# Yaling-Li/DMA-YOLO

Measured on AMD Instinct MI355X. Metric: train images/sec (fwd+loss+bwd+optimizer, train.py batch loop) @1536; detect p50 ms incl. NMS, higher is better.
Workload: dtype bf16; 1 GPU; yolov5l-ca-sppfcspc-bifpn-scconv.yaml train @1536 nc=10; model=yolov5l-ca-sppfcspc-bifpn-scconv.yaml, global_batch=32, img=1536, parallelism=dp1

## Files before the change

### dma-yolo_amd/csrc/bn.hip

```cpp
#include "launch.h"

namespace {

template <typename T>
__global__ void bn_stats_kernel(const T* __restrict__ z, long zps, long M, int C, int rows_per_block,
                                float* __restrict__ psum, float* __restrict__ psq) {
  const int c = blockIdx.y * 64 + (threadIdx.x & 63);
  const int ty = threadIdx.x >> 6;
  __shared__ float s1[4][64], s2[4][64];
  float a = 0.f, b = 0.f;
  if (c < C) {
    const long r0 = (long)blockIdx.x * rows_per_block;
    const long r1 = min(M, r0 + rows_per_block);
#pragma unroll 8
    for (long m = r0 + ty; m < r1; m += 4) {
      float v = to_f(z[m * zps + c]);
      a += v;
      b += v * v;
    }
  }
  s1[ty][threadIdx.x & 63] = a;
  s2[ty][threadIdx.x & 63] = b;
  __syncthreads();
  if (ty == 0 && c < C) {
    const int l = threadIdx.x;
    psum[(long)blockIdx.x * C + c] = s1[0][l] + s1[1][l] + s1[2][l] + s1[3][l];
    psq[(long)blockIdx.x * C + c] = s2[0][l] + s2[1][l] + s2[2][l] + s2[3][l];
  }
}

__global__ void bn_finalize_kernel(const float* __restrict__ psum, const float* __restrict__ psq, int P, int C,
                                   double count, const float* __restrict__ gamma, const float* __restrict__ beta,
                                   float* __restrict__ rmean, float* __restrict__ rvar, long long* nbt, float momentum,
                                   float eps, int update, float* __restrict__ mean, float* __restrict__ invstd,
                                   float* __restrict__ scale, float* __restrict__ shift) {
  const int c = blockIdx.x;
  __shared__ double sa[256], sb[256];
  double a = 0.0, b = 0.0;
#pragma unroll 8
  for (int p = threadIdx.x; p < P; p += blockDim.x) {
    a += (double)psum[(long)p * C + c];
    b += (double)psq[(long)p * C + c];
  }
  sa[threadIdx.x] = a;
  sb[threadIdx.x] = b;
  __syncthreads();
  for (int s = blockDim.x / 2; s > 0; s >>= 1) {
    if ((int)threadIdx.x < s) {
      sa[threadIdx.x] += sa[threadIdx.x + s];
      sb[threadIdx.x] += sb[threadIdx.x + s];
    }
    __syncthreads();
  }
  if (threadIdx.x == 0) {
    const double mu = sa[0] / count;
    double var = sb[0] / count - mu * mu;
    if (var < 0) var = 0;
    const float is = (float)(1.0 / sqrt(var + (double)eps));
    mean[c] = (float)mu;
    invstd[c] = is;
    const float g = gamma ? gamma[c] : 1.f, bb = beta ? beta[c] : 0.f;
    scale[c] = g * is;
    shift[c] = bb - (float)mu * g * is;
    if (update) {
      const double unb = count > 1 ? var * count / (count - 1) : var;
      rmean[c] = (1.f - momentum) * rmean[c] + momentum * (float)mu;
      rvar[c] = (1.f - momentum) * rvar[c] + momentum * (float)unb;
      if (c == 0 && nbt) *nbt += 1;
    }
  }
}

__global__ void bn_eval_coef_kernel(const float* gamma, const float* beta, const float* rmean, const float* rvar,
                                    float eps, int C, float* scale, float* shift) {
  const int c = blockIdx.x * blockDim.x + threadIdx.x;
  if (c >= C) return;
  const float is = 1.f / sqrtf(rvar[c] + eps);
  const float g = gamma ? gamma[c] : 1.f, b = beta ? beta[c] : 0.f;
  scale[c] = g * is;
  shift[c] = b - rmean[c] * g * is;
}

struct RowMap {
  int cv, rr, RB, CV;
  DEV RowMap(int C, int VW) {
    CV = C / VW;
    RB = 256 / CV;
    cv = threadIdx.x % CV;
    rr = threadIdx.x / CV;
  }
  DEV bool active() const { return rr < RB; }
};

template <typename T, int U = 1>
__global__ void __launch_bounds__(256) bn_act_fwd_vec(const T* __restrict__ z, long zps, const float* __restrict__ scale,
                                                      const float* __restrict__ shift, int act, const T* __restrict__ res,
                                                      long rps, T* __restrict__ y, long yps, long M, int C, int rev) {
  constexpr int VW = Traits<T>::VW;
  RowMap rm(C, VW);
  if (!rm.active()) return;
  const int c0 = rm.cv * VW;
  float sc[VW], sh[VW];
  ldf<VW>(scale + c0, sc);
  ldf<VW>(shift + c0, sh);
  const long S = (long)gridDim.x * rm.RB;
  for (long m = (long)blockIdx.x * rm.RB + rm.rr; m < M; m += S * U) {
    uint4 zv[U], rv[U];
#pragma unroll
    for (int u = 0; u < U; ++u) {
      const long mu = rev ? M - 1 - (m + u * S) : m + u * S;
      if (m + u * S < M) {
        zv[u] = *reinterpret_cast<const uint4*>(z + mu * zps + c0);
        if (res) rv[u] = *reinterpret_cast<const uint4*>(res + mu * rps + c0);
      }
    }
#pragma unroll
    for (int u = 0; u < U; ++u) {
      const long mu = rev ? M - 1 - (m + u * S) : m + u * S;
      if (m + u * S >= M) break;
      float f[VW];
      unpack<T>(zv[u], f);
#pragma unroll
      for (int j = 0; j < VW; ++j) f[j] = f[j] * sc[j] + sh[j];
      act_fwd_n<VW>(act, f);
      if (res) {
        float r[VW];
        unpack<T>(rv[u], r);
#pragma unroll
        for (int j = 0; j < VW; ++j) f[j] += r[j];
      }
      *reinterpret_cast<uint4*>(y + mu * yps + c0) = pack<T>(f);
    }
  }
}

__global__ void __launch_bounds__(256) bn_act_fwd_f8_kernel(const bf16* __restrict__ z, long zps,
                                                            const float* __restrict__ scale,
                                                            const float* __restrict__ shift, int act,
                                                            const bf16* __restrict__ res, long rps, bf16* __restrict__ y,
                                                            long yps, long M, int C, unsigned char* __restrict__ y8,
                                                            const float* __restrict__ pmax, int G,
                                                            float* __restrict__ nmax, float* __restrict__ used,
                                                            float headroom, float* __restrict__ nsat) {
  __shared__ float red[4], rsat[4];
  float a = 0.f;
  for (int i = threadIdx.x; i < G; i += 256) a = nanmax(a, pmax[i]);
#pragma unroll
  for (int o = 32; o > 0; o >>= 1) a = nanmax(a, __shfl_xor(a, o, 64));
  if ((threadIdx.x & 63) == 0) red[threadIdx.x >> 6] = a;
  __syncthreads();
  a = nanmax(nanmax(red[0], red[1]), nanmax(red[2], red[3]));
  __syncthreads();
  a *= headroom;
  if (blockIdx.x == 0 && threadIdx.x == 0) used[0] = a;
  const float inv = a > 0.f ? 448.f / a : 1.f, thr = a > 0.f ? a : 448.f;
  RowMap rm(C, 8);
  float mx = 0.f, sat = 0.f;
  if (rm.active()) {
    const int c0 = rm.cv * 8;
    float sc[8], sh[8];
    ldf<8>(scale + c0, sc);
    ldf<8>(shift + c0, sh);
    for (long m = (long)blockIdx.x * rm.RB + rm.rr; m < M; m += (long)gridDim.x * rm.RB) {
      float f[8];
      unpack<bf16>(*reinterpret_cast<const uint4*>(z + m * zps + c0), f);
#pragma unroll
      for (int j = 0; j < 8; ++j) f[j] = f[j] * sc[j] + sh[j];
      act_fwd_n<8>(act, f);
      if (res) {
        float r[8];
        unpack<bf16>(*reinterpret_cast<const uint4*>(res + m * rps + c0), r);
#pragma unroll
        for (int j = 0; j < 8; ++j) f[j] += r[j];
      }
      const uint4 v = pack<bf16>(f);
      *reinterpret_cast<uint4*>(y + m * yps + c0) = v;
      unpack<bf16>(v, f);
#pragma unroll
      for (int j = 0; j < 8; ++j) {
        mx = nanmax(mx, fabsf(f[j]));
        sat += fabsf(f[j]) > thr ? 1.f : 0.f;
      }
      uint2 o;
      o.x = pack4_e4m3(f[0] * inv, f[1] * inv, f[2] * inv, f[3] * inv);
      o.y = pack4_e4m3(f[4] * inv, f[5] * inv, f[6] * inv, f[7] * inv);
      *reinterpret_cast<uint2*>(y8 + m * C + c0) = o;
    }
  }
#pragma unroll
  for (int o = 32; o > 0; o >>= 1) mx = nanmax(mx, __shfl_xor(mx, o, 64));
#pragma unroll
  for (int o = 32; o > 0; o >>= 1) sat += __shfl_xor(sat, o, 64);
  if ((threadIdx.x & 63) == 0) {
    red[threadIdx.x >> 6] = mx;
    rsat[threadIdx.x >> 6] = sat;
  }
  __syncthreads();
  if (threadIdx.x == 0) {
    nmax[blockIdx.x] = nanmax(nanmax(red[0], red[1]), nanmax(red[2], red[3]));
    if (nsat) nsat[blockIdx.x] = (rsat[0] + rsat[1]) + (rsat[2] + rsat[3]);
  }
}

template <typename T>
__global__ void bn_act_fwd_scalar(const T* __restrict__ z, long zps, const float* __restrict__ scale,
                                  const float* __restrict__ shift, int act, const T* __restrict__ res, long rps,
                                  T* __restrict__ y, long yps, long M, int C) {
  const long total = M * C;
  for (long i = blockIdx.x * (long)blockDim.x + threadIdx.x; i < total; i += (long)gridDim.x * blockDim.x) {
    const long m = i / C;
    const int c = (int)(i % C);
    float v = act_fwd(act, to_f(z[m * zps + c]) * scale[c] + shift[c]);
    if (res) v += to_f(res[m * rps + c]);
    y[m * yps + c] = from_f<T>(v);
  }
}

template <typename T, bool STATS, int U = 1>
__global__ void __launch_bounds__(256) bn_bwd_reduce_vec(const T* __restrict__ z, long zps, const T* __restrict__ dy,
                                                         long dps, const float* __restrict__ scale,
                                                         const float* __restrict__ shift, const float* __restrict__ mean,
                                                         const float* __restrict__ invstd, int act, long M, int C,
                                                         float* __restrict__ pdb, float* __restrict__ pdg, int rev) {
  constexpr int VW = Traits<T>::VW;
  __shared__ float red[2][256 * VW];
  RowMap rm(C, VW);
  const int c0 = rm.cv * VW;
  float a[VW], b[VW];
#pragma unroll
  for (int j = 0; j < VW; ++j) { a[j] = 0.f; b[j] = 0.f; }
  if (rm.active()) {
    float sc[VW], sh[VW], mu[VW], is[VW];
    if (STATS) {
#pragma unroll
      for (int j = 0; j < VW; ++j) {
        sc[j] = 1.f;
        sh[j] = 0.f;
        mu[j] = 0.f;
        is[j] = 1.f;
      }
    } else {
      ldf<VW>(scale + c0, sc);
      ldf<VW>(shift + c0, sh);
      ldf<VW>(mean + c0, mu);
      ldf<VW>(invstd + c0, is);
    }
    const long S = (long)gridDim.x * rm.RB;
    for (long m = (long)blockIdx.x * rm.RB + rm.rr; m < M; m += S * U) {
      uint4 zv[U], gv[U];
#pragma unroll
      for (int u = 0; u < U; ++u) {
        const long mu = rev ? M - 1 - (m + u * S) : m + u * S;
        if (m + u * S < M) {
          zv[u] = *reinterpret_cast<const uint4*>(z + mu * zps + c0);
          if (!STATS) gv[u] = *reinterpret_cast<const uint4*>(dy + mu * dps + c0);
        }
      }
#pragma unroll
      for (int u = 0; u < U; ++u) {
        if (m + u * S >= M) break;
        float zf[VW], gf[VW];
        unpack<T>(zv[u], zf);
        if (!STATS) unpack<T>(gv[u], gf);
        if (STATS) {
#pragma unroll
          for (int j = 0; j < VW; ++j) {
            a[j] += zf[j];
            b[j] += zf[j] * zf[j];
          }
        } else {
          float ag[VW];
#pragma unroll
          for (int j = 0; j < VW; ++j) ag[j] = zf[j] * sc[j] + sh[j];
          act_grad_n<VW>(act, ag);
#pragma unroll
          for (int j = 0; j < VW; ++j) {
            const float du = gf[j] * ag[j];
            a[j] += du;
            b[j] += du * (zf[j] - mu[j]) * is[j];
          }
        }
      }
    }
  }
#pragma unroll
  for (int j = 0; j < VW; ++j) {
    red[0][threadIdx.x * VW + j] = a[j];
    red[1][threadIdx.x * VW + j] = b[j];
  }
  __syncthreads();
  for (int c = threadIdx.x; c < C; c += blockDim.x) {
    const int cv = c / VW, j = c % VW;
    float s1 = 0.f, s2 = 0.f;
    for (int r = 0; r < rm.RB; ++r) {
      const int t = r * rm.CV + cv;
      s1 += red[0][t * VW + j];
      s2 += red[1][t * VW + j];
    }
    pdb[(long)blockIdx.x * C + c] = s1;
    pdg[(long)blockIdx.x * C + c] = s2;
  }
}

template <typename T, int U = 1>
__global__ void __launch_bounds__(256) bn_bwd_apply_vec(const T* __restrict__ z, long zps, const T* __restrict__ dy,
                                                        long dps, const float* __restrict__ scale,
                                                        const float* __restrict__ shift, const float* __restrict__ mean,
                                                        const float* __restrict__ invstd, int act,
                                                        const float* __restrict__ ca, const float* __restrict__ cb,
                                                        const float* __restrict__ cc, T* __restrict__ dz, long dzps,
                                                        long M, int C, int rev) {
  constexpr int VW = Traits<T>::VW;
  RowMap rm(C, VW);
  if (!rm.active()) return;
  const int c0 = rm.cv * VW;
  float sc[VW], sh[VW], k1[VW], k0[VW], k2[VW], t0[VW], t1[VW];
  ldf<VW>(scale + c0, sc);
  ldf<VW>(shift + c0, sh);
  ldf<VW>(ca + c0, k1);
  ldf<VW>(cc + c0, k2);
  ldf<VW>(invstd + c0, t0);
  ldf<VW>(cb + c0, k0);
  ldf<VW>(mean + c0, t1);
#pragma unroll
  for (int j = 0; j < VW; ++j) {
    k2[j] = k2[j] * t0[j];
    k0[j] = k0[j] - k2[j] * t1[j];
  }
  const long S = (long)gridDim.x * rm.RB;
  for (long m = (long)blockIdx.x * rm.RB + rm.rr; m < M; m += S * U) {
    uint4 zv[U], gv[U];
#pragma unroll
    for (int u = 0; u < U; ++u) {
      const long mu = rev ? M - 1 - (m + u * S) : m + u * S;
      if (m + u * S < M) {
        zv[u] = *reinterpret_cast<const uint4*>(z + mu * zps + c0);
        gv[u] = *reinterpret_cast<const uint4*>(dy + mu * dps + c0);
      }
    }
#pragma unroll
    for (int u = 0; u < U; ++u) {
      const long mu = rev ? M - 1 - (m + u * S) : m + u * S;
      if (m + u * S >= M) break;
      float zf[VW], gf[VW], o[VW];
      unpack<T>(zv[u], zf);
      unpack<T>(gv[u], gf);
#pragma unroll
      for (int j = 0; j < VW; ++j) o[j] = zf[j] * sc[j] + sh[j];
      act_grad_n<VW>(act, o);
#pragma unroll
      for (int j = 0; j < VW; ++j) o[j] = k1[j] * (gf[j] * o[j]) + k0[j] + k2[j] * zf[j];
      *reinterpret_cast<uint4*>(dz + mu * dzps + c0) = pack<T>(o);
    }
  }
}

template <typename T>
__global__ void bn_bwd_apply_scalar(const T* __restrict__ z, long zps, const T* __restrict__ dy, long dps,
                                    const float* __restrict__ scale, const float* __restrict__ shift,
                                    const float* __restrict__ mean, const float* __restrict__ invstd, int act,
                                    const float* __restrict__ ca, const float* __restrict__ cb,
                                    const float* __restrict__ cc, T* __restrict__ dz, long dzps, long M, int C) {
  const long total = M * C;
  for (long i = blockIdx.x * (long)blockDim.x + threadIdx.x; i < total; i += (long)gridDim.x * blockDim.x) {
    const long m = i / C;
    const int c = (int)(i % C);
    const float zv = to_f(z[m * zps + c]);
    const float du = to_f(dy[m * dps + c]) * act_grad(act, zv * scale[c] + shift[c]);
    dz[m * dzps + c] = from_f<T>(ca[c] * du + cb[c] + cc[c] * (zv - mean[c]) * invstd[c]);
  }
}

template <typename T>
__global__ void bn_bwd_reduce_kernel(const T* __restrict__ z, long zps, const T* __restrict__ dy, long dps,
                                     const float* __restrict__ scale, const float* __restrict__ shift,
                                     const float* __restrict__ mean, const float* __restrict__ invstd, int act,
                                     long M, int C, int rows_per_block, float* __restrict__ pdb,
                                     float* __restrict__ pdg) {
  const int c = blockIdx.y * 64 + (threadIdx.x & 63);
  const int ty = threadIdx.x >> 6;
  __shared__ float s1[4][64], s2[4][64];
  float a = 0.f, b = 0.f;
  if (c < C) {
    const float sc = scale[c], sh = shift[c], mu = mean[c], is = invstd[c];
    const long r0 = (long)blockIdx.x * rows_per_block;
    const long r1 = min(M, r0 + rows_per_block);
    for (long m = r0 + ty; m < r1; m += 4) {
      const float zv = to_f(z[m * zps + c]);
      const float du = to_f(dy[m * dps + c]) * act_grad(act, zv * sc + sh);
      a += du;
      b += du * (zv - mu) * is;
    }
  }
  s1[ty][threadIdx.x & 63] = a;
  s2[ty][threadIdx.x & 63] = b;
  __syncthreads();
  if (ty == 0 && c < C) {
    const int l = threadIdx.x;
    pdb[(long)blockIdx.x * C + c] = s1[0][l] + s1[1][l] + s1[2][l] + s1[3][l];
    pdg[(long)blockIdx.x * C + c] = s2[0][l] + s2[1][l] + s2[2][l] + s2[3][l];
  }
}

__global__ void bn_bwd_finalize_kernel(const float* __restrict__ pdb, const float* __restrict__ pdg, int P, int C,
                                       double count, const float* __restrict__ gamma, const float* __restrict__ invstd,
                                       float* __restrict__ dgamma, float* __restrict__ dbeta, float* __restrict__ ca,
                                       float* __restrict__ cb, float* __restrict__ cc) {
  const int c = blockIdx.x;
  __shared__ double sa[256], sb[256];
  double a = 0.0, b = 0.0;
#pragma unroll 8
  for (int p = threadIdx.x; p < P; p += blockDim.x) {
    a += (double)pdb[(long)p * C + c];
    b += (double)pdg[(long)p * C + c];
  }
  sa[threadIdx.x] = a;
  sb[threadIdx.x] = b;
  __syncthreads();
  for (int s = blockDim.x / 2; s > 0; s >>= 1) {
    if ((int)threadIdx.x < s) {
      sa[threadIdx.x] += sa[threadIdx.x + s];
      sb[threadIdx.x] += sb[threadIdx.x + s];
    }
    __syncthreads();
  }
  if (threadIdx.x == 0) {
    const float db = (float)sa[0], dg = (float)sb[0];
    if (dbeta) dbeta[c] = db;
    if (dgamma) dgamma[c] = dg;
    const float g = gamma ? gamma[c] : 1.f;
    const float k = g * invstd[c];
    ca[c] = k;
    cb[c] = (float)(-(double)k * sa[0] / count);
    cc[c] = (float)(-(double)k * sb[0] / count);
  }
}

__global__ void colsum2_kernel(const float* __restrict__ a, const float* __restrict__ b, long P, int C, int rows_per,
                               float* __restrict__ oa, float* __restrict__ ob) {
  const int c = blockIdx.y * 64 + (threadIdx.x & 63);
  const int ty = threadIdx.x >> 6;
  __shared__ double s1[4][64], s2[4][64];
  double x = 0.0, y = 0.0;
  if (c < C) {
    const long r0 = (long)blockIdx.x * rows_per, r1 = min(P, r0 + rows_per);
#pragma unroll 8
    for (long r = r0 + ty; r < r1; r += 4) {
      x += a[r * C + c];
      y += b[r * C + c];
    }
  }
  s1[ty][threadIdx.x & 63] = x;
  s2[ty][threadIdx.x & 63] = y;
  __syncthreads();
  if (ty == 0 && c < C) {
    const int l = threadIdx.x;
    oa[(long)blockIdx.x * C + c] = (float)(s1[0][l] + s1[1][l] + s1[2][l] + s1[3][l]);
    ob[(long)blockIdx.x * C + c] = (float)(s2[0][l] + s2[1][l] + s2[2][l] + s2[3][l]);
  }
}

}

constexpr int kRevAct = 1, kRevReduce = 0, kRevApply = 1;

DMY_API int dmy_bn_partial_rows(long M) {
  long p = (M + 255) / 256;
  return (int)(p < 1024 ? (p < 1 ? 1 : p) : 1024);
}

DMY_API int dmy_bn_stats(int dtype, const void* z, long zps, long M, int C, float* psum, float* psq, void* stream) {
  return by_dtype(dtype, kInvalid, [&](auto tag) {
    using T = typename decltype(tag)::type;
    constexpr int VW = Traits<T>::VW;
    hipStream_t st = (hipStream_t)stream;
    if (vec_ok(VW, C, {zps}, {}, {z}) && C / VW <= 256) {
      bn_bwd_reduce_vec<T, true><<<row_grid(M, C, VW, kRedCap), 256, 0, st>>>(
          (const T*)z, zps, (const T*)z, zps, nullptr, nullptr, nullptr, nullptr, 0, M, C, psum, psq, 0);
    } else {
      const int P = dmy_bn_partial_rows(M);
      const int rpb = (int)((M + P - 1) / P);
      bn_stats_kernel<T><<<dim3(P, ceil_div(C, 64)), 256, 0, st>>>((const T*)z, zps, M, C, rpb, psum, psq);
    }
    return (int)hipGetLastError();
  });
}

DMY_API int dmy_bn_finalize(const float* psum, const float* psq, int P, int C, double count, const float* gamma,
                            const float* beta, float* rmean, float* rvar, long long* nbt, float momentum, float eps,
                            int update, float* mean, float* invstd, float* scale, float* shift, void* stream) {
  bn_finalize_kernel<<<C, 256, 0, (hipStream_t)stream>>>(psum, psq, P, C, count, gamma, beta, rmean, rvar, nbt,
                                                         momentum, eps, update, mean, invstd, scale, shift);
  return (int)hipGetLastError();
}

DMY_API int dmy_bn_eval_coef(const float* gamma, const float* beta, const float* rmean, const float* rvar, float eps,
                             int C, float* scale, float* shift, void* stream) {
  bn_eval_coef_kernel<<<ceil_div(C, 256), 256, 0, (hipStream_t)stream>>>(gamma, beta, rmean, rvar, eps, C, scale, shift);
  return (int)hipGetLastError();
}


DMY_API int dmy_bn_act_fwd(int dtype, const void* z, long zps, const float* scale, const float* shift, int act,
                           const void* res, long rps, void* y, long yps, long M, int C, void* stream) {
  return by_dtype(dtype, kInvalid, [&](auto tag) {
    using T = typename decltype(tag)::type;
    constexpr int VW = Traits<T>::VW;
    hipStream_t st = (hipStream_t)stream;
    if (vec_ok(VW, C, {zps, yps, res ? rps : 0}, {}, {z, y, res}) && C / VW <= 256)
      bn_act_fwd_vec<T><<<row_grid(M, C, VW, kEwCap), 256, 0, st>>>((const T*)z, zps, scale, shift, act, (const T*)res, rps,
                                                                    (T*)y, yps, M, C, kRevAct);
    else
      bn_act_fwd_scalar<T><<<grid_cap(ceil_div(M * C, 256), 8192), 256, 0, st>>>((const T*)z, zps, scale, shift, act,
                                                                                 (const T*)res, rps, (T*)y, yps, M, C);
    return (int)hipGetLastError();
  });
}

DMY_API int dmy_bn_act_f8_blocks(void) { return 1024; }

DMY_API int dmy_bn_act_fwd_f8(const void* z, long zps, const float* scale, const float* shift, int act, const void* res,
                              long rps, void* y, long yps, long M, int C, void* y8, const float* pmax, float* nmax,
                              float* used, float headroom, float* nsat, void* stream) {
  if (C / 8 > 256 || !vec_ok(8, C, {zps, yps, res ? rps : 0}, {}, {z, y, res}) || ((uintptr_t)y8 & 7) || !(headroom >= 1.f))
    return kInvalid;
  const int G = dmy_bn_act_f8_blocks();
  bn_act_fwd_f8_kernel<<<G, 256, 0, (hipStream_t)stream>>>((const bf16*)z, zps, scale, shift, act, (const bf16*)res, rps,
                                                          (bf16*)y, yps, M, C, (unsigned char*)y8, pmax, G, nmax, used,
                                                          headroom, nsat);
  return (int)hipGetLastError();
}

DMY_API int dmy_bn_reduce_rows(int dtype, const void* z, long zps, const void* dy, long dps, long M, int C) {
  const int VW = vec_width(dtype);
  if (vec_ok(VW, C, {zps, dy ? dps : 0}, {}, {z, dy}) && C / VW <= 256) return row_grid(M, C, VW, kRedCap);
  return dmy_bn_partial_rows(M);
}

DMY_API int dmy_bn_bwd_reduce(int dtype, const void* z, long zps, const void* dy, long dps, const float* scale,
                              const float* shift, const float* mean, const float* invstd, int act, long M, int C,
                              float* pdb, float* pdg, void* stream) {
  return by_dtype(dtype, kInvalid, [&](auto tag) {
    using T = typename decltype(tag)::type;
    constexpr int VW = Traits<T>::VW;
    hipStream_t st = (hipStream_t)stream;
    if (vec_ok(VW, C, {zps, dps}, {}, {z, dy}) && C / VW <= 256) {
      bn_bwd_reduce_vec<T, false><<<row_grid(M, C, VW, kRedCap), 256, 0, st>>>(
          (const T*)z, zps, (const T*)dy, dps, scale, shift, mean, invstd, act, M, C, pdb, pdg, kRevReduce);
    } else {
      const int P = dmy_bn_partial_rows(M);
      const int rpb = (int)((M + P - 1) / P);
      bn_bwd_reduce_kernel<T><<<dim3(P, ceil_div(C, 64)), 256, 0, st>>>((const T*)z, zps, (const T*)dy, dps, scale, shift,
                                                                        mean, invstd, act, M, C, rpb, pdb, pdg);
    }
    return (int)hipGetLastError();
  });
}

DMY_API int dmy_colsum2_rows(long P) { return (int)(P < 256 ? P : 256); }

DMY_API int dmy_colsum2(const float* a, const float* b, long P, int C, float* oa, float* ob, void* stream) {
  const int S = dmy_colsum2_rows(P);
  const int rows = (int)((P + S - 1) / S);
  dim3 grid(S, ceil_div(C, 64));
  colsum2_kernel<<<grid, 256, 0, (hipStream_t)stream>>>(a, b, P, C, rows, oa, ob);
  return (int)hipGetLastError();
}

DMY_API int dmy_bn_bwd_finalize(const float* pdb, const float* pdg, int P, int C, double count, const float* gamma,
                                const float* invstd, float* dgamma, float* dbeta, float* ca, float* cb, float* cc,
                                void* stream) {
  bn_bwd_finalize_kernel<<<C, 256, 0, (hipStream_t)stream>>>(pdb, pdg, P, C, count, gamma, invstd, dgamma, dbeta, ca,
                                                             cb, cc);
  return (int)hipGetLastError();
}

DMY_API int dmy_bn_bwd_apply(int dtype, const void* z, long zps, const void* dy, long dps, const float* scale,
                             const float* shift, const float* mean, const float* invstd, int act, const float* ca,
                             const float* cb, const float* cc, void* dz, long dzps, long M, int C, void* stream) {
  return by_dtype(dtype, kInvalid, [&](auto tag) {
    using T = typename decltype(tag)::type;
    constexpr int VW = Traits<T>::VW;
    hipStream_t st = (hipStream_t)stream;
    if (vec_ok(VW, C, {zps, dps, dzps}, {}, {z, dy, dz}) && C / VW <= 256)
      bn_bwd_apply_vec<T><<<row_grid(M, C, VW, kEwCap), 256, 0, st>>>((const T*)z, zps, (const T*)dy, dps, scale, shift, mean,
                                                                      invstd, act, ca, cb, cc, (T*)dz, dzps, M, C, kRevApply);
    else
      bn_bwd_apply_scalar<T><<<grid_cap(ceil_div(M * C, 256), 8192), 256, 0, st>>>(
          (const T*)z, zps, (const T*)dy, dps, scale, shift, mean, invstd, act, ca, cb, cc, (T*)dz, dzps, M, C);
    return (int)hipGetLastError();
  });
}

__global__ void reduce_rows_kernel(const float* __restrict__ part, int P, int C, float* __restrict__ out, int acc) {
  const int c = blockIdx.x;
  __shared__ double s[256];
  double a = 0.0;
#pragma unroll 8
  for (int p = threadIdx.x; p < P; p += blockDim.x) a += (double)part[(long)p * C + c];
  s[threadIdx.x] = a;
  __syncthreads();
  for (int k = blockDim.x / 2; k > 0; k >>= 1) {
    if ((int)threadIdx.x < k) s[threadIdx.x] += s[threadIdx.x + k];
    __syncthreads();
  }
  if (threadIdx.x == 0) out[c] = (acc ? out[c] : 0.f) + (float)s[0];
}

DMY_API int dmy_reduce_rows(const float* part, int P, int C, float* out, int accumulate, void* stream) {
  reduce_rows_kernel<<<C, 256, 0, (hipStream_t)stream>>>(part, P, C, out, accumulate);
  return (int)hipGetLastError();
}

namespace {
DEV void pix_hwb(long m, int W, int H, bool small, int& w, int& h, int& b) {
  if (small) {
    const unsigned u = (unsigned)m, q = u / (unsigned)W;
    w = (int)(u - q * (unsigned)W);
    b = (int)(q / (unsigned)H);
    h = (int)(q - (unsigned)b * (unsigned)H);
  } else {
    w = (int)(m % W);
    h = (int)((m / W) % H);
    b = (int)(m / ((long)W * H));
  }
}

DEV int nearest_src_bn(int d, int in, int out) {
  if (out == in) return d;
  if (out == 2 * in) return d >> 1;
  const float scale = (float)in / (float)out;
  const int s = (int)floorf(__fmul_rn((float)d, scale));
  return s < in - 1 ? s : in - 1;
}

__global__ void __launch_bounds__(256) scgate_bn_fwd_kernel(const bf16* __restrict__ x, long xps,
                                                            const bf16* __restrict__ z, const float* __restrict__ scale,
                                                            const float* __restrict__ shift, const bf16* __restrict__ g,
                                                            bf16* __restrict__ out, int N, int H, int W, int C, int GH,
                                                            int GW) {
  constexpr int VW = 8;
  RowMap rm(C, VW);
  if (!rm.active()) return;
  const int c0 = rm.cv * VW;
  float sc[VW], sh[VW];
  ldf<VW>(scale + c0, sc);
  ldf<VW>(shift + c0, sh);
  const long M = (long)N * H * W, S = (long)gridDim.x * rm.RB;
  const bool small = M < (1L << 31);
  for (long m = (long)blockIdx.x * rm.RB + rm.rr; m < M; m += S) {
    int w, h, b;
    pix_hwb(m, W, H, small, w, h, b);
    const long gp = ((long)b * GH + nearest_src_bn(h, GH, H)) * GW + nearest_src_bn(w, GW, W);
    const uint4 xv = *reinterpret_cast<const uint4*>(x + m * xps + c0);
    const uint4 zv = *reinterpret_cast<const uint4*>(z + m * C + c0);
    const uint4 gv = *reinterpret_cast<const uint4*>(g + gp * C + c0);
    float xf[VW], zf[VW], gf[VW], o[VW];
    unpack<bf16>(xv, xf);
    unpack<bf16>(zv, zf);
    unpack<bf16>(gv, gf);
#pragma unroll
    for (int j = 0; j < VW; ++j) {
      const float u = to_f(from_f<bf16>(zf[j] * sc[j] + sh[j]));
      const float sg = sigmoidf_(to_f(from_f<bf16>(xf[j] + gf[j])));
      o[j] = u * to_f(from_f<bf16>(sg));
    }
    *reinterpret_cast<uint4*>(out + m * C + c0) = pack<bf16>(o);
  }
}

__global__ void __launch_bounds__(256) scgate_bn_bwd_kernel(
    const bf16* __restrict__ x, long xps, const bf16* __restrict__ z, const float* __restrict__ scale,
    const float* __restrict__ shift, const float* __restrict__ mean, const float* __restrict__ invstd,
    const bf16* __restrict__ g, const bf16* __restrict__ dout, bf16* __restrict__ du3, bf16* __restrict__ dpre, int N,
    int H, int W, int C, int GH, int GW, float* __restrict__ pdb, float* __restrict__ pdg) {
  constexpr int VW = 8;
  __shared__ float red[2][256 * VW];
  RowMap rm(C, VW);
  const int c0 = rm.cv * VW;
  float a[VW], bsum[VW];
#pragma unroll
  for (int j = 0; j < VW; ++j) a[j] = bsum[j] = 0.f;
  if (rm.active()) {
    float sc[VW], sh[VW], mu[VW], is[VW];
    ldf<VW>(scale + c0, sc);
    ldf<VW>(shift + c0, sh);
    ldf<VW>(mean + c0, mu);
    ldf<VW>(invstd + c0, is);
    const long M = (long)N * H * W, S = (long)gridDim.x * rm.RB;
    const bool small = M < (1L << 31);
    for (long m = (long)blockIdx.x * rm.RB + rm.rr; m < M; m += S) {
      int w, h, b;
      pix_hwb(m, W, H, small, w, h, b);
      const long gp = ((long)b * GH + nearest_src_bn(h, GH, H)) * GW + nearest_src_bn(w, GW, W);
      const uint4 xv = *reinterpret_cast<const uint4*>(x + m * xps + c0);
      const uint4 zv = *reinterpret_cast<const uint4*>(z + m * C + c0);
      const uint4 gv = *reinterpret_cast<const uint4*>(g + gp * C + c0);
      const uint4 dv = *reinterpret_cast<const uint4*>(dout + m * C + c0);
      float xf[VW], zf[VW], gf[VW], df[VW], du[VW], dp[VW];
      unpack<bf16>(xv, xf);
      unpack<bf16>(zv, zf);
      unpack<bf16>(gv, gf);
      unpack<bf16>(dv, df);
#pragma unroll
      for (int j = 0; j < VW; ++j) {
        const float u = to_f(from_f<bf16>(zf[j] * sc[j] + sh[j]));
        const float sg = sigmoidf_(to_f(from_f<bf16>(xf[j] + gf[j])));
        dp[j] = df[j] * u * sg * (1.f - sg);
        du[j] = df[j] * sg;
      }
      const uint4 duv = pack<bf16>(du);
      *reinterpret_cast<uint4*>(du3 + m * C + c0) = duv;
      *reinterpret_cast<uint4*>(dpre + m * C + c0) = pack<bf16>(dp);
      float dr[VW];
      unpack<bf16>(duv, dr);
#pragma unroll
      for (int j = 0; j < VW; ++j) {
        a[j] += dr[j];
        bsum[j] += dr[j] * (zf[j] - mu[j]) * is[j];
      }
    }
  }
#pragma unroll
  for (int j = 0; j < VW; ++j) {
    red[0][threadIdx.x * VW + j] = a[j];
// ... 44 lines not shown
```

### dma-yolo_amd/csrc/bwd1x1.hip

```cpp
#include "launch.h"

namespace {
namespace b1 {

constexpr unsigned kOob = 0xFFFFFFF0u;

DEV __amdgpu_buffer_rsrc_t rsrc(const void* base, unsigned bytes) {
  return __builtin_amdgcn_make_buffer_rsrc(const_cast<void*>(base), 0, (int)bytes, 0x00020000);
}
DEV uint4 bload(__amdgpu_buffer_rsrc_t r, unsigned off) {
  const auto v = __builtin_amdgcn_raw_buffer_load_b128(r, off, 0, 0);
  return *reinterpret_cast<const uint4*>(&v);
}

template <int ROW> DEV int ksw(int k, int row) {
  constexpr int RB = ROW * 2;
  const int c = row >> 3, w = row & 7;
  int key;
  if constexpr (RB >= 256) key = 2 * ((k & 3) | (((k >> 3) & 1) << 2));
  else key = 2 * (((k >> 1) & 1) | (((k >> 3) & 1) << 1));
  return k * ROW + (((c ^ key) & (ROW / 8 - 1)) << 3) + w;
}
template <int K> DEV int wsw(int r, int ch) {
  if constexpr (K * 2 >= 256) return (ch ^ (r & 15)) & (K / 8 - 1);
  else return (ch ^ ((r >> 1) & 7)) & (K / 8 - 1);
}
template <int ROW> DEV bf16x8 frag_t(const bf16* base, int r0, int k0, int lane) {
  typedef short s4 __attribute__((ext_vector_type(4)));
  const int g = lane >> 4, il = lane & 15, q = il >> 2, p = il & 3;
  const bf16* a0 = base + ksw<ROW>(k0 + 8 * g + q, r0 + 4 * p);
  const bf16* a1 = base + ksw<ROW>(k0 + 8 * g + 4 + q, r0 + 4 * p);
  const s4 lo = __builtin_amdgcn_ds_read_tr16_b64_v4i16((__attribute__((address_space(3))) s4*)(a0));
  const s4 hi = __builtin_amdgcn_ds_read_tr16_b64_v4i16((__attribute__((address_space(3))) s4*)(a1));
  bf16x8 r;
  r[0] = lo[0]; r[1] = lo[1]; r[2] = lo[2]; r[3] = lo[3];
  r[4] = hi[0]; r[5] = hi[1]; r[6] = hi[2]; r[7] = hi[3];
  return r;
}
DEV unsigned pk2(float a, float b) {
  const bf16 x = __float2bfloat16(a), y = __float2bfloat16(b);
  return (unsigned)*reinterpret_cast<const unsigned short*>(&x) |
         ((unsigned)*reinterpret_cast<const unsigned short*>(&y) << 16);
}

template <int K, int CB, int TP, int PX>
struct Shape {
  static constexpr int NT = 256, KCH = K / 8, CCH = CB / 8;
  static constexpr int NDZ = TP * KCH / NT, NX = TP * CCH / NT;
  static constexpr int RDZ = NT / KCH, RXS = NT / CCH;
  static constexpr int KW = K / 2, CW = CB / 2, MI = KW / 16, NJ = CW / 16;
  static constexpr int PGN = TP / (16 * PX), U = PGN * (CB / 64), UPW = (U + 3) / 4;
  static constexpr int LDS = (CB * K + TP * K + TP * CB) * 2;
  static_assert(K % 64 == 0 && CB % 64 == 0 && NT % KCH == 0 && NT % CCH == 0, "channels");
  static_assert(NDZ >= 1 && NX >= 1 && TP % 32 == 0 && TP % (16 * PX) == 0 && U >= 1, "tile");
  static_assert(LDS <= 160 * 1024, "LDS");
};

template <int K, int CB, int TP, int PX>
__global__ void __launch_bounds__(256, 1) conv1x1_bwd_bn(
    const bf16* __restrict__ dy, long dps, const bf16* __restrict__ z, const bf16* __restrict__ x, long xps,
    const bf16* __restrict__ wt, const float* __restrict__ scale, const float* __restrict__ shift,
    const float* __restrict__ mean, const float* __restrict__ invstd, int act, const float* __restrict__ ca,
    const float* __restrict__ cb, const float* __restrict__ cc, bf16* __restrict__ dx, long bps, int accumulate,
    float* __restrict__ dw, float* __restrict__ dws, long M, int ntiles, int C, int nsplit, unsigned dyb, unsigned zb,
    unsigned xb) {
  using S = Shape<K, CB, TP, PX>;
  extern __shared__ __attribute__((aligned(16))) char b1_smem[];
  bf16* ws = reinterpret_cast<bf16*>(b1_smem);
  bf16* dzs = ws + CB * K;
  bf16* xs = dzs + TP * K;
  const int tid = threadIdx.x, lane = tid & 63, wid = tid >> 6, g = lane >> 4, il = lane & 15;
  const int slot = blockIdx.x >> 3, cs = slot % nsplit;
  const int grp = (blockIdx.x & 7) + 8 * (slot / nsplit), ngrp = gridDim.x / nsplit;
  const int cbase = cs * CB;
  x += cbase;
  dx += cbase;
  dw += cbase;

  for (int e = tid; e < CB * S::KCH; e += S::NT) {
    const int r = e / S::KCH, ch = e % S::KCH;
    *reinterpret_cast<uint4*>(ws + r * K + (wsw<K>(r, ch) << 3)) =
        *reinterpret_cast<const uint4*>(wt + (long)(cbase + r) * K + ch * 8);
  }

  const int kc8 = (tid % S::KCH) * 8, xc8 = (tid % S::CCH) * 8;
  float sc[8], sh[8], k1[8], k0[8], k2[8];
  {
    float t0[8], t1[8];
    ldf<8>(scale + kc8, sc);
    ldf<8>(shift + kc8, sh);
    ldf<8>(ca + kc8, k1);
    ldf<8>(cc + kc8, k2);
    ldf<8>(invstd + kc8, t0);
    ldf<8>(cb + kc8, k0);
    ldf<8>(mean + kc8, t1);
#pragma unroll
    for (int j = 0; j < 8; ++j) {
      k2[j] = k2[j] * t0[j];
      k0[j] = k0[j] - k2[j] * t1[j];
    }
  }

  const __amdgpu_buffer_rsrc_t rdy = rsrc(dy, dyb), rz = rsrc(z, zb), rx = rsrc(x, xb - 2u * cbase);
  uint4 pg[S::NDZ], pz[S::NDZ], pxv[S::NX];
  auto issue = [&](int t) {
    const long m0 = (long)t * TP;
#pragma unroll
    for (int j = 0; j < S::NDZ; ++j) {
      const long m = m0 + tid / S::KCH + j * S::RDZ;
      const bool ok = m < M;
      pg[j] = bload(rdy, ok ? (unsigned)((m * dps + kc8) * 2) : kOob);
      pz[j] = bload(rz, ok ? (unsigned)((m * K + kc8) * 2) : kOob);
    }
#pragma unroll
    for (int j = 0; j < S::NX; ++j) {
      const long m = m0 + tid / S::CCH + j * S::RXS;
      pxv[j] = bload(rx, m < M ? (unsigned)((m * xps + xc8) * 2) : kOob);
    }
  };

  f32x4 wacc[S::MI][S::NJ];
#pragma unroll
  for (int i = 0; i < S::MI; ++i)
#pragma unroll
    for (int j = 0; j < S::NJ; ++j) wacc[i][j] = f32x4{0.f, 0.f, 0.f, 0.f};
  const int wk = wid >> 1, wc = wid & 1;
  const int chq = (g & 1) * 16 + (g >> 1) * 8;

  int t = grp;
  if (t < ntiles) issue(t);
  __syncthreads();
  for (; t < ntiles; t += ngrp) {
    const long m0 = (long)t * TP;
#pragma unroll
    for (int j = 0; j < S::NDZ; ++j) {
      float zf[8], gf[8], o[8];
      unpack<bf16>(pz[j], zf);
      unpack<bf16>(pg[j], gf);
#pragma unroll
      for (int e = 0; e < 8; ++e) o[e] = zf[e] * sc[e] + sh[e];
      act_grad_n<8>(act, o);
#pragma unroll
      for (int e = 0; e < 8; ++e) o[e] = k1[e] * (gf[e] * o[e]) + k0[e] + k2[e] * zf[e];
      pg[j] = pack<bf16>(o);
    }
    __syncthreads();
#pragma unroll
    for (int j = 0; j < S::NDZ; ++j)
      *reinterpret_cast<uint4*>(dzs + ksw<K>(tid / S::KCH + j * S::RDZ, kc8)) = pg[j];
#pragma unroll
    for (int j = 0; j < S::NX; ++j)
      *reinterpret_cast<uint4*>(xs + ksw<CB>(tid / S::CCH + j * S::RXS, xc8)) = pxv[j];
    __syncthreads();

    uint4 old[S::UPW][PX][2];
    if (accumulate) {
#pragma unroll
      for (int s = 0; s < S::UPW; ++s) {
        const int u = wid + 4 * s, p0 = (u % S::PGN) * 16 * PX, c0 = (u / S::PGN) * 64;
        if (u >= S::U) break;
#pragma unroll
        for (int pt = 0; pt < PX; ++pt) {
          const long m = m0 + p0 + pt * 16 + il;
#pragma unroll
          for (int h = 0; h < 2; ++h)
            old[s][pt][h] = m < M ? *reinterpret_cast<const uint4*>(dx + m * bps + c0 + h * 32 + chq)
                                  : make_uint4(0, 0, 0, 0);
        }
      }
    }
    if (t + ngrp < ntiles) issue(t + ngrp);

#pragma unroll
    for (int s = 0; s < S::UPW; ++s) {
      const int u = wid + 4 * s, p0 = (u % S::PGN) * 16 * PX, c0 = (u / S::PGN) * 64;
      if (u >= S::U) break;
      f32x4 acc[4][PX];
#pragma unroll
      for (int ct = 0; ct < 4; ++ct)
#pragma unroll
        for (int pt = 0; pt < PX; ++pt) acc[ct][pt] = f32x4{0.f, 0.f, 0.f, 0.f};
#pragma unroll 2
      for (int kc = 0; kc < K / 32; ++kc) {
        bf16x8 b[PX];
#pragma unroll
        for (int pt = 0; pt < PX; ++pt)
          b[pt] = *reinterpret_cast<const bf16x8*>(dzs + ksw<K>(p0 + pt * 16 + il, kc * 32 + 8 * g));
#pragma unroll
        for (int ct = 0; ct < 4; ++ct) {
          const int r = c0 + ct * 16 + il;
          const bf16x8 a = *reinterpret_cast<const bf16x8*>(ws + r * K + (wsw<K>(r, kc * 4 + g) << 3));
#pragma unroll
          for (int pt = 0; pt < PX; ++pt)
            acc[ct][pt] = __builtin_amdgcn_mfma_f32_16x16x32_bf16(a, b[pt], acc[ct][pt], 0, 0, 0);
        }
      }
#pragma unroll
      for (int pt = 0; pt < PX; ++pt) {
        const long m = m0 + p0 + pt * 16 + il;
#pragma unroll
        for (int h = 0; h < 2; ++h) {
          const f32x4 &a = acc[2 * h][pt], &b = acc[2 * h + 1][pt];
          const auto s0 = __builtin_amdgcn_permlane16_swap(pk2(a[0], a[1]), pk2(b[0], b[1]), false, false);
          const auto s1 = __builtin_amdgcn_permlane16_swap(pk2(a[2], a[3]), pk2(b[2], b[3]), false, false);
          uint4 v;
          v.x = s0[0];
          v.y = s1[0];
          v.z = s0[1];
          v.w = s1[1];
          if (accumulate) {
            float f[8], o[8];
            unpack<bf16>(v, f);
            unpack<bf16>(old[s][pt][h], o);
#pragma unroll
            for (int j = 0; j < 8; ++j) f[j] += o[j];
            v = pack<bf16>(f);
          }
          if (m < M) *reinterpret_cast<uint4*>(dx + m * bps + c0 + h * 32 + chq) = v;
        }
      }
    }

#pragma unroll
    for (int ps = 0; ps < TP / 32; ++ps) {
      bf16x8 a[S::MI];
#pragma unroll
      for (int i = 0; i < S::MI; ++i) a[i] = frag_t<K>(dzs, wk * S::KW + i * 16, ps * 32, lane);
#pragma unroll
      for (int j = 0; j < S::NJ; ++j) {
        const bf16x8 b = frag_t<CB>(xs, wc * S::CW + j * 16, ps * 32, lane);
#pragma unroll
        for (int i = 0; i < S::MI; ++i)
          wacc[i][j] = __builtin_amdgcn_mfma_f32_16x16x32_bf16(a[i], b, wacc[i][j], 0, 0, 0);
      }
    }
  }
  float* part = dws != nullptr ? dws + (long)blockIdx.x * K * CB : nullptr;
#pragma unroll
  for (int i = 0; i < S::MI; ++i)
#pragma unroll
    for (int j = 0; j < S::NJ; ++j)
#pragma unroll
      for (int r = 0; r < 4; ++r) {
        const int kk = wk * S::KW + i * 16 + 4 * g + r, c = wc * S::CW + j * 16 + il;
        if (part != nullptr) part[kk * CB + c] = wacc[i][j][r];
        else atomicAdd(dw + (long)kk * C + c, wacc[i][j][r]);
      }
}

__global__ void __launch_bounds__(256) wgrad_slots_reduce(const float* __restrict__ dws, float* __restrict__ dw, int K,
                                                          int C, int CB, int nblocks, int nsplit) {
  const long e = (long)blockIdx.x * blockDim.x + threadIdx.x;
  if (e >= (long)K * C) return;
  const int k = (int)(e / C), c = (int)(e % C), cs = c / CB, cl = c % CB;
  float s = 0.f;
  for (int b = 0; b < nblocks; ++b)
    if (((b >> 3) % nsplit) == cs) s += dws[((long)b * K + k) * CB + cl];
  dw[e] += s;
}

int num_cus() {
  static int n = 0;
  if (n == 0) {
    int dev = 0;
    (void)hipGetDevice(&dev);
    if (hipDeviceGetAttribute(&n, hipDeviceAttributeMultiprocessorCount, dev) != hipSuccess || n <= 0) n = 256;
  }
  return n;
}

struct Plan {
  int cb, tp, px;
};
constexpr Plan plan(int K, int C) {
  return (K == 64 && C == 64) ? Plan{64, 128, 2} : (K == 128 && C == 64) ? Plan{64, 128, 2}
       : (K == 64 && C == 128) ? Plan{128, 64, 2} : (K == 128 && C == 128) ? Plan{128, 64, 2}
       : (K == 128 && C == 256) ? Plan{256, 64, 2} : (K == 128 && C == 512) ? Plan{256, 64, 2}
       : (K == 256 && C == 256) ? Plan{128, 32, 1} : (K == 256 && C == 128) ? Plan{128, 32, 1}
       : (K == 64 && C == 256) ? Plan{256, 64, 2} : Plan{0, 0, 0};
}

inline int grid_blocks(long M, int K, int C) {
  const Plan pl = plan(K, C);
  const int ns = C / pl.cb, ntiles = ceil_div(M, pl.tp);
  int ngrp = num_cus() / ns;
  if (ngrp > ntiles) ngrp = (ntiles + 7) / 8 * 8;
  return ngrp * ns;
}

template <int K, int C>
int launch(const bf16* dy, long dps, const bf16* z, const bf16* x, long xps, const bf16* wt, const float* scale,
           const float* shift, const float* mean, const float* invstd, int act, const float* ca, const float* cb,
           const float* cc, bf16* dx, long bps, int acc, float* dw, float* ws, long M, hipStream_t st) {
  constexpr Plan pl = plan(K, C);
  constexpr int CB = pl.cb, TP = pl.tp, PX = pl.px, NS = C / CB;
  using S = Shape<K, CB, TP, PX>;
  static bool raised = false;
  if (!raised) {
    (void)hipFuncSetAttribute((const void*)conv1x1_bwd_bn<K, CB, TP, PX>,
                              hipFuncAttributeMaxDynamicSharedMemorySize, S::LDS);
    raised = true;
  }
  const int nb = grid_blocks(M, K, C);
  conv1x1_bwd_bn<K, CB, TP, PX><<<nb, 256, S::LDS, st>>>(
      dy, dps, z, x, xps, wt, scale, shift, mean, invstd, act, ca, cb, cc, dx, bps, acc, dw, ws, M, ceil_div(M, TP), C,
      NS, (unsigned)(2.0 * (double)M * dps), (unsigned)(2.0 * (double)M * K), (unsigned)(2.0 * (double)M * xps));
  if (ws != nullptr)
    wgrad_slots_reduce<<<ceil_div((long)K * C, 256), 256, 0, st>>>(ws, dw, K, C, CB, nb, NS);
  return (int)hipGetLastError();
}
}
}

DMY_API int dmy_conv1x1_bwd_bn_ok(long M, int K, int C, long dps, long xps, long bps, const void* dy, const void* z,
                                  const void* x, const void* dx) {
  if (b1::plan(K, C).cb == 0 || M <= 0) return 0;
  if (!vec_ok(8, 0, {dps, xps, bps}, {}, {dy, z, x, dx}) || dps < K || xps < C || bps < C) return 0;
  const double lim = (double)b1::kOob - 64.0;
  if (2.0 * (double)M * dps >= lim || 2.0 * (double)M * K >= lim || 2.0 * (double)M * xps >= lim) return 0;
  return 1;
}

DMY_API long dmy_conv1x1_bwd_bn_ws_elems(long M, int K, int C) {
  if (b1::plan(K, C).cb == 0 || M <= 0) return 0;
  return (long)b1::grid_blocks(M, K, C) * K * b1::plan(K, C).cb;
}

DMY_API int dmy_conv1x1_bwd_bn(const void* dy, long dps, const void* z, const void* x, long xps, const void* wt,
                               const float* scale, const float* shift, const float* mean, const float* invstd, int act,
                               const float* ca, const float* cb, const float* cc, void* dx, long bps, int accumulate,
                               float* dw, float* ws, long ws_elems, long M, int K, int C, void* stream) {
  if (!dmy_conv1x1_bwd_bn_ok(M, K, C, dps, xps, bps, dy, z, x, dx)) return -1;
  if (ws != nullptr && ws_elems < dmy_conv1x1_bwd_bn_ws_elems(M, K, C)) return -1;
  hipStream_t st = (hipStream_t)stream;
#define B1_GO(K_, C_)                                                                                                 \
  if (K == K_ && C == C_)                                                                                            \
    return b1::launch<K_, C_>((const bf16*)dy, dps, (const bf16*)z, (const bf16*)x, xps, (const bf16*)wt, scale,     \
                              shift, mean, invstd, act, ca, cb, cc, (bf16*)dx, bps, accumulate, dw, ws, M, st);
  B1_GO(64, 64)
  B1_GO(128, 64)
  B1_GO(64, 128)
  B1_GO(128, 128)
  B1_GO(128, 256)
  B1_GO(128, 512)
  B1_GO(256, 128)
  B1_GO(256, 256)
  B1_GO(64, 256)
#undef B1_GO
  return -1;
}
```

### dma-yolo_amd/dmayolo/_lib.py

```python
import ctypes
import os

import torch

_HERE = os.path.dirname(os.path.abspath(__file__))
LIB_PATH = os.path.join(_HERE, 'libdmayolo_hip.so')
if os.environ.get('DMY_LIB_AB'):
    LIB_PATH = os.path.join(_HERE, os.path.basename(os.environ['DMY_LIB_AB']))

P, I, L, F, D = ctypes.c_void_p, ctypes.c_int, ctypes.c_long, ctypes.c_float, ctypes.c_double

SIGNATURES = {
    'dmy_conv_fwd_partial_rows': [L, I],
    'dmy_conv_fwd_bound_rows': [L, I],
    'dmy_conv_fwd_last_rows': [],
    'dmy_conv_fwd_bn_rows': [I, P, P, P, P, I, I, I, I, L, I, I, I, I, I, I, I, L],
    'dmy_conv_fwd': [I, P, P, P, P, P, P, I, I, I, I, L, I, I, I, I, I, I, I, L, P],
    'dmy_conv_dgrad': [I, P, P, P, I, I, I, I, I, L, I, I, I, I, I, I, I, L, P],
    'dmy_conv_fwd_act': [I, P, P, P, P, I, I, I, I, L, I, I, I, I, I, I, I, L, P, P, I, P, L, P],
    'dmy_conv_fwd_splitk_elems': [I, P, P, P, I, I, I, I, L, I, I, I, I, I, I, I, L],
    'dmy_conv_fwd_act_ws': [I, P, P, P, P, I, I, I, I, L, I, I, I, I, I, I, I, L, P, P, I, P, L, P, L, P],
    'dmy_conv_route': [I, I, P, P, P, I, I, I, I, L, I, I, I, I, I, I, I, L, I],
    'dmy_conv_wgrad': [I, P, P, P, I, I, I, I, L, I, I, I, I, I, I, I, L, P],
    'dmy_conv_wprep_multi': [I, P, I, P],
    'dmy_conv_wprep_s2d': [I, P, P, I, I, I, P],
    'dmy_conv_wgrad_s2d_to_oihw': [P, P, I, I, I, P],
    'dmy_image_s2d': [I, I, P, P, I, I, I, I, I, F, P],
    'dmy_conv_wgrad_ex': [I, P, P, P, I, I, I, I, L, I, I, I, I, I, I, I, L, I, P],
    'dmy_conv_wgrad_ws_elems': [I, P, P, I, I, I, I, L, I, I, I, I, I, I, I, L, I],
    'dmy_conv_wgrad_det': [I, P, P, P, I, I, I, I, L, I, I, I, I, I, I, I, L, I, P, L, P],
    'dmy_conv_wprep': [I, P, P, P, I, I, I, I, I, P],
    'dmy_dwconv_ok': [I, P, P, P, I, I, I, I, I, I, L, I, I, I, I, I, I, L],
    'dmy_dwconv_fwd_rows': [L, I],
    'dmy_dwconv_fwd': [I, P, P, P, P, P, P, I, I, I, I, L, I, I, I, I, I, I, L, P],
    'dmy_dwconv_fwd_act': [I, P, P, P, P, I, I, I, I, L, I, I, I, I, I, I, L, P, P, I, P, L, P],
    'dmy_dwconv_dgrad': [I, P, P, P, I, I, I, I, I, L, I, I, I, I, I, I, L, P],
    'dmy_dwconv_wgrad_rows': [L, I],
    'dmy_dwconv_wgrad': [I, P, P, P, I, I, I, I, L, I, I, I, I, I, I, L, P],
    'dmy_dwconv_wgrad_finalize': [P, I, I, I, I, P, I, P],
    'dmy_dwconv_wgrad_bias': [I, P, P, P, I, I, I, I, L, I, I, I, I, I, I, L, P],
    'dmy_dwconv_wgrad_bias_finalize': [P, I, I, I, I, P, I, P, I, P],
    'dmy_dwconv_fwd_actbn': [I, P, P, P, P, I, I, I, I, L, I, I, I, I, I, I, L, P, P, I, P, L, P],
    'dmy_actbn_stats': [I, P, L, I, L, I, P, P, P],
    'dmy_actbn_fwd': [I, P, L, I, P, P, P, L, P, L, L, I, P],
    'dmy_actbn_bwd_reduce': [I, P, L, P, L, P, P, I, L, I, P, P, P],
    'dmy_actbn_bwd_apply': [I, P, L, P, L, P, P, I, P, P, P, P, L, L, I, P, P],
    'dmy_adapt_gate_blocks': [I, L, I, I],
    'dmy_adapt_gate_fwd': [I, I, P, L, I, P, L, I, P, L, I, P, L, P, P, P, L, P, L, P],
    'dmy_adapt_gate_bwd': [I, I, P, L, P, L, I, P, L, I, P, L, I, P, P, L, P, P, L, P, L, P, L, I, P, L, P, P, L, P],
    'dmy_adapt_add_fwd': [I, I, P, L, P, L, P, L, P, F, P, L, L, I, P],
    'dmy_adapt_add_bwd': [I, I, P, L, P, L, P, L, P, L, P, F, P, L, P, L, P, L, I, P, L, I, P],
    'dmy_conv1x1_bwd_bn_ok': [L, I, I, L, L, L, P, P, P, P],
    'dmy_conv1x1_bwd_bn': [P, L, P, P, L, P, P, P, P, P, I, P, P, P, P, L, I, P, P, L, L, I, I, P],
    'dmy_conv1x1_bwd_bn_ws_elems': [L, I, I],
    'dmy_aug_desc_bytes': [],
    'dmy_augment_batch': [P, I, P, I, I, P],
    'dmy_mosaic_desc_bytes': [],
    'dmy_mosaic_compose': [P, I, I, P],
    'dmy_letterbox_desc_bytes': [],
    'dmy_letterbox_batch': [I, P, P, I, P, I, I, I, I, F, P],
    'dmy_scale_boxes': [P, P, P, P, P, P, I, I, P],
    'dmy_fp8_quant_ws_elems': [],
    'dmy_fp8_quant': [P, L, I, L, P, P, P],
    'dmy_conv_wprep_fp8': [P, P, P, I, I, I, I, P],
    'dmy_conv_fwd_fp8_partial_rows': [L, I],
    'dmy_conv_fwd_fp8': [P, P, P, P, P, P, P, P, I, I, I, I, I, I, I, I, I, I, I, L, P, P, I, P, L, P],
    'dmy_conv_wgrad_to_oihw': [P, P, I, I, I, I, I, P],
    'dmy_bn_partial_rows': [L],
    'dmy_bn_stats': [I, P, L, L, I, P, P, P],
    'dmy_bn_finalize': [P, P, I, I, D, P, P, P, P, P, F, F, I, P, P, P, P, P],
    'dmy_bn_eval_coef': [P, P, P, P, F, I, P, P, P],
    'dmy_bn_act_fwd': [I, P, L, P, P, I, P, L, P, L, L, I, P],
    'dmy_bn_act_f8_blocks': [],
    'dmy_bn_act_fwd_f8': [P, L, P, P, I, P, L, P, L, L, I, P, P, P, P, F, P, P],
    'dmy_bn_bwd_reduce': [I, P, L, P, L, P, P, P, P, I, L, I, P, P, P],
    'dmy_bn_bwd_finalize': [P, P, I, I, D, P, P, P, P, P, P, P, P],
    'dmy_bn_bwd_apply': [I, P, L, P, L, P, P, P, P, I, P, P, P, P, L, L, I, P],
    'dmy_reduce_rows': [P, I, I, P, I, P],
    'dmy_bn_reduce_rows': [I, P, L, P, L, L, I],
    'dmy_colsum2_rows': [L],
    'dmy_colsum2': [P, P, L, I, P, P, P],
    'dmy_bn_act_s2d_fwd': [I, P, L, P, P, I, P, L, I, I, I, I, P],
    'dmy_bn_bwd_reduce_s2d_rows': [I, L, I],
    'dmy_bn_bwd_reduce_s2d': [I, P, L, P, L, P, P, P, P, I, I, I, I, I, P, P, P],
    'dmy_bn_bwd_apply_s2d': [I, P, L, P, L, P, P, P, P, I, P, P, P, P, L, I, I, I, I, P],
    'dmy_maxpool2_fwd': [I, P, L, P, L, P, I, I, I, I, P],
    'dmy_maxpool2_bwd': [I, P, L, P, P, L, I, I, I, I, I, P],
    'dmy_spd_split_fwd': [I, P, L, P, L, P, L, P, I, I, I, I, P],
    'dmy_spd_split_bwd': [I, P, L, P, L, P, P, L, I, I, I, I, P],
    'dmy_gate_fwd': [I, P, L, P, L, P, L, L, I, F, P],
    'dmy_gate_bwd': [I, P, L, P, L, P, L, P, L, P, L, L, I, F, P],
    'dmy_layerscale_fwd': [I, P, L, P, P, P, L, L, I, P],
    'dmy_layerscale_bwd_rows': [L],
    'dmy_layerscale_bwd': [I, P, L, P, P, P, L, I, P, P],
    'dmy_maxpool_fwd': [I, P, L, P, L, P, I, I, I, I, I, P],
    'dmy_maxpool_chain3_fwd': [I, P, L, P, P, P, L, I, I, I, I, I, P],
    'dmy_maxpool_bwd': [I, P, L, P, P, L, I, I, I, I, I, I, P],
    'dmy_avgpool_fwd': [I, P, L, P, I, I, I, I, I, P],
    'dmy_avgpool_bwd': [I, P, P, L, I, I, I, I, I, I, P],
    'dmy_resize_fwd': [I, P, L, P, L, F, I, I, I, I, I, I, P],
    'dmy_resize_bwd': [I, P, L, P, L, I, I, I, I, I, I, P],
    'dmy_slice_copy': [I, P, L, P, L, L, I, P, I, I, F, I, P],
    'dmy_slice_copy_dot': [I, P, L, P, L, P, L, L, I, P, I, I, F, I, P, P],
    'dmy_dot_partial_blocks': [L, I],
    'dmy_dot_partial': [I, P, L, P, L, L, I, P, P],
    'dmy_bifpn_wgrad': [P, I, I, P, F, P, P],
    'dmy_scgate_fwd': [I, P, L, P, P, P, I, I, I, I, I, I, P],
    'dmy_scgate_bwd': [I, P, L, P, P, P, P, P, L, I, I, I, I, I, I, I, P],
    'dmy_scgate_bn_rows': [I, I, I, I],
    'dmy_scgate_bn_fwd': [P, L, P, P, P, P, P, I, I, I, I, I, I, P],
    'dmy_scgate_bn_bwd': [P, L, P, P, P, P, P, P, P, P, P, I, I, I, I, I, I, P, P, P],
    'dmy_ca_pool_fwd': [I, P, L, P, I, I, I, I, P],
    'dmy_ca_pool_bwd': [I, P, P, L, I, I, I, I, I, P],
    'dmy_ca_apply_fwd': [I, P, L, P, P, P, L, I, I, I, I, P],
    'dmy_ca_apply_bwd': [I, P, L, P, P, P, L, P, L, P, P, I, I, I, I, P],
    'dmy_nchw_to_nhwc': [I, I, P, P, I, I, I, I, I, F, P],
    'dmy_nhwc_to_nchw_f32': [I, P, L, P, I, I, I, I, P],
    'dmy_pointwise': [I, I, I, P, P, P, L, F, P],
    'dmy_cast': [I, I, P, P, L, F, P],
    'dmy_tta_image': [I, I, P, P, I, I, I, I, I, I, F, I, I, I, I, I, F, P],
    'dmy_detect_decode': [I, P, L, L, L, I, I, I, I, I, F, P, P, L, L, P],
    'dmy_detect_decode_levels': [I, I, P, P, P, P, I, I, I, P, P, L, P],
    'dmy_detect_decode_tta': [I, I, P, P, P, P, I, I, I, P, P, L, F, I, F, F, I, L, P],
    'dmy_build_targets': [P, I, P, I, I, I, F, P, P, P, P, P, P, P, P, P],
    'dmy_yolo_loss_part_rows': [],
    'dmy_yolo_loss_level': [I, P, L, L, L, L, I, I, I, I, I, I, F, F, F, F, F, F, F, F, F, P, P, P, P, P, P, P, P,
                            I, P, P, P, P, P, P],
    'dmy_yolo_loss_finalize': [P, I, F, F, F, F, P, P, P],
    'dmy_yolo_loss_level_focal': [I, P, L, L, L, L, I, I, I, I, I, I, F, F, F, F, F, F, F, P, I, F, F, P, P, P, P, P,
                                  P, P, P, I, P, P, P, P, P, P],
    'dmy_yolo_loss_finalize_balance': [P, I, F, F, F, F, P, I, I, P, P, P],
    'dmy_loss_grad': [I, P, P, P, L, P],
    'dmy_siou_eval': [P, P, P, P, I, P],
    'dmy_tal_workspace_bytes': [I, I, I],
    'dmy_tal_loss': [I, P, L, L, L, P, L, L, L, I, I, I, P, P, P, P, I, F, F, F, P, P, P, P, P],
    'dmy_tal_flatten': [I, P, L, I, I, I, I, I, I, P, I, P],
    'dmy_tal_detect_out': [I, P, I, I, I, P, P, P, P, P],
    'dmy_space_to_depth': [I, P, L, P, L, I, I, I, I, I, P],
    'dmy_gpool_ws_bytes': [I, I, I, I],
    'dmy_gpool_fwd': [I, P, L, I, I, I, P, P, P, P],
    'dmy_gpool_bwd': [I, P, P, P, L, I, I, I, I, P],
    'dmy_halves_sigmoid': [I, P, I, I, P, P, P, P],
    'dmy_cbam_in_fwd': [I, P, L, P, I, I, I, P, P, P, P],
    'dmy_cbam_in_bwd_ws_elems': [I, I, I],
    'dmy_cbam_in_bwd': [I, P, L, P, P, L, P, P, I, I, I, P, L, I, P, P, P],
    'dmy_pixscale': [I, P, P, L, I, I, I, P, L, P, L, P, P, P],
    'dmy_mha_fwd': [I, P, L, P, L, P, L, P, L, P, I, I, I, I, F, P],
    'dmy_mha_fwd_ref': [I, P, L, P, L, P, L, P, L, P, I, I, I, I, F, P],
    'dmy_mha_bwd': [I, P, L, P, L, P, L, P, P, L, P, P, P, P, P, I, I, I, I, F, P],
    'dmy_dropout_seed': [P, P, P],
    'dmy_dropout': [I, P, L, P, L, L, I, F, P, P],
    'dmy_nms_candidates': [P, I, I, I, F, I, P, P, L, P, P],
    'dmy_nms_sort': [P, L, P, I, P],
    'dmy_nms_greedy': [P, I, I, I, F, I, I, I, P, L, P, P, P, P, P, P],
    'dmy_nms_mask_rows': [],
    'dmy_nms_greedy_mask': [P, I, I, I, F, I, I, I, P, L, P, P, P, P, P, P, P],
    'dmy_wbf_max_rows': [],
    'dmy_wbf_workspace_bytes': [I, I],
    'dmy_wbf': [P, P, P, P, I, I, I, D, D, P, P, P, P],
    'dmy_process_batch': [P, P, P, P, I, P, I, P, P, P, P, P],
    'dmy_layernorm_fwd': [I, P, L, P, P, P, P, P, L, I, F, P],
    'dmy_layernorm_bwd_blocks': [L],
    'dmy_layernorm_bwd': [I, P, L, P, L, P, P, P, P, L, I, L, I, P, P, P],
    'dmy_winattn_fwd': [I, P, P, P, I, I, I, I, I, I, F, P],
    'dmy_winattn_bwd_groups': [I, I, I, I],
    'dmy_winattn_bwd': [I, P, P, P, P, P, P, I, I, I, I, I, I, F, P],
    'dmy_sample_scale': [I, P, P, P, L, L, P],
    'dmy_droppath_add': [I, P, P, P, F, P, L, L, P],
    'dmy_droppath_grad': [I, P, P, F, P, L, L, P],
}


KERN = {n: i for i, n in enumerate(
    ['HALO', 'SPLITK', 'P1S', 'STEM', 'P1P', 'PIPE8', 'WIDE', 'WIDE288', 'TALL', 'V3', 'V2',
     'V2_BIG', 'S2_Q2S', 'S2_Q2', 'S2_MERGED', 'S2_CLASS',
     'W_TAP128', 'W_TAP64', 'W_TAP64X2', 'W_V4', 'W_V3', 'W_V3N128', 'W_V3N256', 'W_V2_128', 'W_V2_64'])}
ROUTE_FWD, ROUTE_DGRAD, ROUTE_WGRAD = 0, 1, 2

SELF_BOUND = {'dmy_chunk_size', 'dmy_sgd', 'dmy_adam', 'dmy_ema', 'dmy_amp_check', 'dmy_amp_update'}
LONG_RET = {'dmy_conv_fwd_bound_rows', 'dmy_conv_fwd_last_rows'}


def restype(name):
    return ctypes.c_long if name.endswith(('_bytes', '_elems')) or name in LONG_RET else ctypes.c_int


class LibraryMissing(RuntimeError):
    pass


def _load():
    if not os.path.exists(LIB_PATH):
        raise LibraryMissing(f'{LIB_PATH} not built: run `python -c "import __graft_entry__ as g; g.build()"` '
                             '(the DMA-YOLO HIP path has no CPU fallback)')
    lib = ctypes.CDLL(LIB_PATH)
    for name, argt in SIGNATURES.items():
        fn = getattr(lib, name)
        fn.argtypes = argt
        fn.restype = restype(name)
    return lib


lib = _load()


def call(name, *args):
    rc = getattr(lib, name)(*args)
    if name.endswith(('_rows', '_blocks', '_groups', '_bytes', '_elems', '_ok', '_route')):
        return rc
    if rc != 0:
        raise RuntimeError(f'{name} failed with hipError {rc}')
    return rc


_raw_stream = getattr(torch._C, '_cuda_getCurrentRawStream', None)


def stream():
    if _raw_stream is not None:
        return ctypes.c_void_p(_raw_stream(torch.cuda.current_device()))
    return ctypes.c_void_p(torch.cuda.current_stream().cuda_stream)


def ptr(t):
    return None if t is None else ctypes.c_void_p(t.data_ptr())


ACT_NONE, ACT_SILU, ACT_HARDSWISH, ACT_SIGMOID, ACT_GELU, ACT_RELU, ACT_LEAKY = 0, 1, 2, 3, 4, 5, 6
```

### dma-yolo_amd/dmayolo/functional.py

```python
import os
import weakref
from collections import namedtuple

import torch

from . import _lib
from ._lib import call, ptr, stream, ACT_NONE, ACT_SILU, ACT_HARDSWISH, ACT_SIGMOID, ACT_GELU, ACT_RELU, ACT_LEAKY

DT = {torch.float32: 0, torch.bfloat16: 1}
CL = torch.channels_last


def dcode(t):
    try:
        return DT[t.dtype]
    except KeyError:
        raise TypeError(f'dmayolo kernels take float32 or bfloat16 activations, got {t.dtype}')


def pixel_stride(t):
    N, C, H, W = t.shape
    for attempt in range(2):
        s = t.stride()
        if C == 1 or s[1] == 1:
# ... 15 lines not shown
_CONST = {}


def const_vec(n, value, dev):
    key = (int(n), float(value), str(dev))
    t = _CONST.get(key)
    if t is None:
        t = torch.full((int(n),), float(value), dtype=torch.float32, device=dev)
        if not torch.cuda.is_current_stream_capturing():
            _CONST[key] = t
    return t


def out_view(o, shape, like):
    if o is None or tuple(o.shape) != tuple(shape) or o.dtype != like.dtype or o.device != like.device:
        return None, None
    t, ps = pixel_stride(o)
    return (o, ps) if t is o else (None, None)


def concat_buffer(N, Ct, H, W, like):
    return new_act(N, Ct, H, W, like)


class GradSink:
    __slots__ = ('n', 'seen', 'buf', 'ps', 'adopt')

    def __init__(self, n, adopt=True):
        self.n, self.seen, self.buf, self.ps, self.adopt = n, 0, None, 0, adopt

    def expect(self, k):
        self.n += k
        return self

    def _tick(self):
        self.seen += 1
        if self.seen < self.n:
            return None
        ret = self.buf
        self.buf, self.seen = None, 0
        return ret

    def target(self, N, C, H, W, like):
        if self.buf is None:
            self.buf, self.ps = new_act(N, C, H, W, like), C
            return self.buf, C, 0
        return self.buf, self.ps, 1

    def peek(self, N, C, H, W):
        return (self.buf, self.ps) if self.buf is not None else None

    def done(self):
        return self._tick()

    def passthrough(self, g):
        g, gps = pixel_stride(g)
        if self.buf is None and self.adopt:
            self.buf, self.ps = g, gps
        else:
            N, C, H, W = g.shape
            acc = int(self.buf is not None)
            if not acc:
                self.buf, self.ps = new_act(N, C, H, W, g), C
            call('dmy_slice_copy', dcode(g), ptr(g), gps, ptr(self.buf), self.ps, N * H * W, C, None, 0, 0, 0.0, acc,
                 stream())
        return self._tick()


def sink_target(sink, N, C, H, W, like):
    if sink is None:
        return new_act(N, C, H, W, like), C, 0
    return sink.target(N, C, H, W, like)


def sink_result(sink, buf):
    return buf if sink is None else sink.done()



WGRAD_OIHW, WGRAD_ZEROED = 1, 2
DETERMINISTIC = [False]


def set_deterministic(on=True):
    DETERMINISTIC[0] = bool(on)


class ConvGeom(namedtuple('ConvGeom', 'N C H W xps K k s p OH OW M Cg Hg Wg kg sg pg Cp s2d groups', defaults=(1,))):
    __slots__ = ()

    def launch(self):
        return self.N, self.Hg, self.Wg, self.Cg, self.xps, self.K, self.kg, self.kg, self.sg, self.pg, self.OH, self.OW

    def tag(self):
        return self.N, self.C, self.H, self.W, self.K, self.k, self.s

    def flops(self):
        return 2.0 * self.M * self.K * (self.C // self.groups) * self.k * self.k

    def dw(self):
        return self.N, self.H, self.W, self.C, self.xps, self.k, self.k, self.s, self.p, self.OH, self.OW


def _wgrad(dt, x, dz, dzps, dw, g, flags):
    kw = dict(tag=g.tag(), nbytes=x.element_size() * (g.N * g.Hg * g.Wg * g.Cg + g.M * g.K) +
              4 * g.K * g.Cg * g.kg * g.kg)
    if DETERMINISTIC[0]:
        ne = call('dmy_conv_wgrad_ws_elems', dt, ptr(x), ptr(dz), *g.launch(), dzps, flags)
        ws = f32(ne, dz.device) if ne else None
        KernelTimer.run('conv_wgrad', g.flops(), 'dmy_conv_wgrad_det', dt, ptr(x), ptr(dz), ptr(dw), *g.launch(), dzps,
                        flags, ptr(ws), ne, stream(), **kw)
    else:
        KernelTimer.run('conv_wgrad', g.flops(), 'dmy_conv_wgrad_ex', dt, ptr(x), ptr(dz), ptr(dw), *g.launch(), dzps,
                        flags, stream(), **kw)


class WgradArena:
    current = None
    ALIGN = 64

    def __init__(self, buf, offsets):
        self.buf, self.offsets, self.taken = buf, offsets, set()

    @classmethod
    def layout(cls, params):
        offs, n = {}, 0
        for q in params:
            if q.dim() >= 1 and q.dtype == torch.float32 and q.requires_grad:
                offs[q.data_ptr()] = (n, q.numel())
                n += -(-q.numel() // cls.ALIGN) * cls.ALIGN
        return offs, n

    def take(self, key, shape):
        o = self.offsets.get(key)
        numel = 1
        for d in shape:
            numel *= d
        if o is None or o[1] != numel or key in self.taken:
            return None
        self.taken.add(key)
        return self.buf[o[0]:o[0] + numel].view(shape)


PARAM_GEN = [0]


class WeightPrep:
    current = None
    ALIGN = 64

    def __init__(self, weights, dtype, dev):
        import numpy as np
        sizes = [-(-w.numel() // self.ALIGN) * self.ALIGN for w in weights]
        self.buf = torch.empty(2 * sum(sizes), dtype=dtype, device=dev)
        self.map, recs, off = {}, [], 0
        for w, n in zip(weights, sizes):
            K, C, KH, KW = w.shape
            wf = self.buf[off:off + w.numel()].view(K, KH * KW * C)
            wt = self.buf[off + n:off + n + w.numel()].view(C, KH * KW * K)
            self.map[w.data_ptr()] = (wf, wt)
            recs.append((w.data_ptr(), wf.data_ptr(), wt.data_ptr(), K, C, KH, KW))
            off += 2 * n
        rec = np.dtype([('w', '<u8'), ('wf', '<u8'), ('wt', '<u8'), ('K', '<i4'), ('C', '<i4'), ('KH', '<i4'),
                        ('KW', '<i4')])
        self.table = torch.from_numpy(np.array(recs, dtype=rec).view(np.uint8)).to(dev)
        self.n, self.dtype = len(recs), dtype

    def launch(self):
        call('dmy_conv_wprep_multi', DT[self.dtype], ptr(self.table), self.n, stream())
        return self

    def get(self, weight, dtype):
        return self.map.get(weight.data_ptr()) if dtype == self.dtype else None


class ConvSpec:
    __slots__ = ('stride', 'pad', 'act', 'bn', 'wcache', 'ecache', 'fp8', 'f8cache', 'f8_emit', 'defer', 'groups',
                 '__weakref__')

    def __init__(self, stride, pad, act, bn=None):
        self.stride, self.pad, self.act, self.bn = int(stride), int(pad), int(act), bn
        self.wcache = self.ecache = self.f8cache = self.f8_emit = None
        self.fp8 = False
        self.defer = False
        self.groups = 1


_SPECS = weakref.WeakKeyDictionary()


def spec_for(owner, stride, pad, act, bn):
    sp = _SPECS.get(owner)
    if sp is None or (sp.stride, sp.pad, sp.act) != (int(stride), int(pad), int(act)) or sp.bn is not bn:
        sp = _SPECS[owner] = ConvSpec(stride, pad, act, bn)
    sp.fp8 = bool(getattr(owner, 'dmy_fp8', False))
    sp.groups = int(getattr(owner, 'groups', 1))
    return sp


_PSPECS = {}


def _param_spec(w, stride, pad, act, bn):
    k = id(w)
    ent = _PSPECS.get(k)
    if ent is None or ent[0]() is not w:
        ent = _PSPECS[k] = (weakref.ref(w, lambda _r, k=k: _PSPECS.pop(k, None)), {})
    key = (int(stride), int(pad), int(act), id(bn))
    sp = ent[1].get(key)
    if sp is None or sp.bn is not bn:
        sp = ent[1][key] = ConvSpec(stride, pad, act, bn)
    return sp


def fp8_eligible(C, K, dtype, rows):
    return dtype == torch.bfloat16 and C % 128 == 0 and K % 8 == 0 and K >= 32 and rows * C < 0xFFFFFFF0


def set_fp8(model, on=True, min_k=3):
    n = 0
    for m in model.modules():
        if isinstance(m, torch.nn.Conv2d) and m.groups == 1 and m.kernel_size[0] >= min_k \
                and fp8_eligible(m.in_channels, m.out_channels, torch.bfloat16, 0):
            m.dmy_fp8 = bool(on)
            n += 1
    PARAM_GEN[0] += 1
    return n


_F8_WS = [0]


def _f8_ws():
    _F8_WS[0] = call('dmy_fp8_quant_ws_elems')
    return _F8_WS[0]


F8_DELAYED = [os.environ.get('DMY_F8_DELAYED', '1') == '1']


F8_HEADROOM = [float(os.environ.get('DMY_F8_HEADROOM', '1'))]


class F8Emit:
    __slots__ = ('buf', 'p', 'valid', 'numel')

    def __init__(self, dev):
        nb = call('dmy_bn_act_f8_blocks')
        self.buf = torch.zeros(3, nb, dtype=torch.float32, device=dev)
        self.p, self.valid, self.numel = 0, False, 0

    def run(self, z, scale, shift, act, res, rps, y, yps, M, K):
        y8 = torch.empty(M * K, dtype=torch.uint8, device=z.device)
        used = f32(1, z.device)
        call('dmy_bn_act_fwd_f8', ptr(z), K, ptr(scale), ptr(shift), act, ptr(res), rps, ptr(y), yps, M, K, ptr(y8),
             ptr(self.buf[self.p]), ptr(self.buf[1 - self.p]), ptr(used), F8_HEADROOM[0], ptr(self.buf[2]), stream())
        self.p ^= 1
        out = (y8, used) if self.valid else None
        self.valid, self.numel = True, M * K
        return out

    def saturated(self):
        n = float(self.buf[2].sum()) if self.valid else 0.0
        return n, n / max(1, self.numel)


def f8_saturation(model):
    out = {}
    for name, mod in model.named_modules():
        if not isinstance(mod, torch.nn.Conv2d):
            continue
        sps = [_SPECS[mod]] if mod in _SPECS else []
        ent = _PSPECS.get(id(mod.weight))
        if ent is not None and ent[0]() is mod.weight:
            sps += list(ent[1].values())
        for sp in sps:
            if isinstance(sp.f8_emit, F8Emit):
                out[name] = sp.f8_emit.saturated()
    return out


def _fp8_weight(weight, spec, wkey, dev):
    K, C, KH, KW = weight.shape
    fc = spec.f8cache
    if fc is not None and fc[0] == wkey:
        return fc[1], fc[2]
    w8 = torch.empty(weight.numel(), dtype=torch.uint8, device=dev)
    ws = f32(K, dev)
    call('dmy_conv_wprep_fp8', ptr(weight.detach().contiguous()), ptr(w8), ptr(ws), K, C, KH, KW, stream())
    spec.f8cache = (wkey, w8, ws)
    return w8, ws


def _fp8_operands(x, xps, weight, spec, wkey, f8in=None):
    if f8in is not None:
        x8, amax = f8in
    else:
        N, C, H, W = x.shape
        rows = N * H * W
        x8 = torch.empty(rows * C, dtype=torch.uint8, device=x.device)
        amax = f32(_F8_WS[0] or _f8_ws(), x.device)
        call('dmy_fp8_quant', ptr(x), rows, C, xps, ptr(x8), ptr(amax), stream())
    return (x8, amax, *_fp8_weight(weight, spec, wkey, x.device))


def prep_weight(w, dtype, need_t, Cp=None):
    K, C, KH, KW = w.shape
    Cp = Cp or C
    wc = w.detach().contiguous()
    wf = torch.empty((K, KH * KW * Cp), dtype=dtype, device=w.device)
    wt = torch.empty((C, KH * KW * K), dtype=dtype, device=w.device) if need_t else None
    call('dmy_conv_wprep', DT[dtype], ptr(wc), ptr(wf), ptr(wt), K, C, Cp, KH, KW, stream())
    return wf, wt


VW = {torch.float32: 4, torch.bfloat16: 8}


def vec_ok(dtype, chans=(), strides=(), tensors=()):
    vw = VW[dtype]
    return not (any(c % vw for c in chans) or any(s % vw for s in strides) or any(t.data_ptr() % 16 for t in tensors))


def vec_check(what, dtype, chans=(), strides=(), tensors=(), max_vecs=None):
    if not vec_ok(dtype, chans, strides, tensors) or (max_vecs and any(c // VW[dtype] > max_vecs for c in chans)):
        raise NotImplementedError(f'{what}: channel counts {list(chans)} / pixel strides {list(strides)} must be '
# ... 391 lines not shown
        dz, dzps = new_act(ctx.g.N, K, ctx.g.OH, ctx.g.OW, z), K
        zero, one = const_vec(K, 0.0, dev), const_vec(K, 1.0, dev)
        call('dmy_bn_bwd_apply', dt, ptr(z), K, ptr(dy), dps, ptr(one), ptr(zero), ptr(zero), ptr(one),
             ctx.spec.act, ptr(one), ptr(zero), ptr(zero), ptr(dz), K, M, K, stream())
    if ctx.has_bias and want_bias:
        P = call('dmy_bn_reduce_rows', dt, ptr(dz), dzps, None, 0, M, K)
        ps_, pq_ = f32(P * K, dev), f32(P * K, dev)
        call('dmy_bn_stats', dt, ptr(dz), dzps, M, K, ptr(ps_), ptr(pq_), stream())
        dbias = _pgrad(ctx, 0, K, dev)
        call('dmy_reduce_rows', ptr(ps_), P, K, ptr(dbias), 0, stream())
    return dz, dzps, dbias


def _dgrad(ctx, dt, dz, dzps, wt, z):
    g = ctx.g
    N, C, H, W, K, k, M = g.N, g.C, g.H, g.W, g.K, g.k, g.M
    if g.Cp != C or g.s2d:
        raise NotImplementedError('input gradient of a channel-padded stem conv')
    buf, bps, acc = sink_target(ctx.xsink, N, C, H, W, z)
    if g.groups != 1:
        _dw_check(dt, buf, wt, dz, g, bps, dzps)
        KernelTimer.run('dwconv_dgrad', g.flops(), 'dmy_dwconv_dgrad', dt, ptr(dz), ptr(wt), ptr(buf), acc, N, H, W, C,
                        bps, k, k, g.s, g.p, g.OH, g.OW, dzps, stream(), tag=g.tag(),
                        nbytes=z.element_size() * (M * C + k * k * C + (1 + acc) * N * H * W * C))
        return sink_result(ctx.xsink, buf)
    KernelTimer.run('conv_dgrad', g.flops(), 'dmy_conv_dgrad', dt, ptr(dz), ptr(wt), ptr(buf), acc, N, H, W, C, bps, K,
                    k, k, g.s, g.p, g.OH, g.OW, dzps, stream(), tag=g.tag(),
                    nbytes=z.element_size() * (M * K + K * C * k * k + (1 + acc) * N * H * W * C))
    return sink_result(ctx.xsink, buf)


def _conv_wgrad(ctx, dt, x, dz, dzps, with_bias=False):
    g = ctx.g
    K, C, k, dev = g.K, g.C, g.k, dz.device
    if g.groups != 1:
        dw, zeroed = _wgrad_target(ctx, (K, 1, k, k), dev)
        _dw_check(dt, x, dz, dz, g, g.xps, dzps)
        P = call('dmy_dwconv_wgrad_rows', g.M, C)
        if with_bias:
            part, dbias = f32(P * (k * k + 1) * C, dev), _pgrad(ctx, 0, K, dev)
            KernelTimer.run('dwconv_wgrad', g.flops(), 'dmy_dwconv_wgrad_bias', dt, ptr(x), ptr(dz), ptr(part), *g.dw(),
                            dzps, stream(), tag=g.tag(),
                            nbytes=x.element_size() * (g.N * g.H * g.W * C + g.M * C) + 4 * (k * k + 1) * C)
            call('dmy_dwconv_wgrad_bias_finalize', ptr(part), P, C, k, k, ptr(dw), int(zeroed), ptr(dbias), 0,
                 stream())
            return dw, dbias
        part = f32(P * k * k * C, dev)
        KernelTimer.run('dwconv_wgrad', g.flops(), 'dmy_dwconv_wgrad', dt, ptr(x), ptr(dz), ptr(part), *g.dw(), dzps,
                        stream(), tag=g.tag(),
                        nbytes=x.element_size() * (g.N * g.H * g.W * C + g.M * C) + 4 * k * k * C)
        call('dmy_dwconv_wgrad_finalize', ptr(part), P, C, k, k, ptr(dw), int(zeroed), stream())
        return dw, None
    dw, zeroed = _wgrad_target(ctx, (K, C, k, k), dev)
    if g.s2d:
        dwo = f32(K * 9 * g.s2d, dev)
        _wgrad(dt, x, dz, dzps, dwo, g, 0)
        call('dmy_conv_wgrad_s2d_to_oihw', ptr(dwo), ptr(dw), K, C, g.s2d, stream())
    elif k == 1 and g.Cp == C:
        _wgrad(dt, x, dz, dzps, dw, g, WGRAD_OIHW | (WGRAD_ZEROED if zeroed else 0))
    else:
        dwo = f32(K * g.Cp * k * k, dev)
        _wgrad(dt, x, dz, dzps, dwo, g, 0)
        call('dmy_conv_wgrad_to_oihw', ptr(dwo), ptr(dw), K, C, g.Cp, k, k, stream())
    return dw, None


class ConvBNActFn(torch.autograd.Function):
    @staticmethod
    def forward(ctx, x, weight, bias, gamma, beta, res, spec, xsink=None, rsink=None, grad_on=True, out=None, spd=False):
        f8in, prod = getattr(x, '_dmy_f8', None), getattr(x, '_dmy_prod', None)
        need_grad = grad_on and any(ctx.needs_input_grad[:6])
        bn = spec.bn
        train_bn = bn is not None and (bn.training or not bn.track_running_stats)
        infer = not need_grad and not train_bn
        x, g, wf, wt, wkey = _conv_operands(x, weight, spec, need_grad, infer)
        f8 = _conv_fp8(x, g, weight, spec, wkey, f8in, prod, infer)
        res, rps = pixel_stride(res) if res is not None else (None, 0)
        oshape = _spd_shape(g, x, res) if spd else (g.N, g.K, g.OH, g.OW)
        act_pass = spd or bn is not None or spec.act != ACT_NONE or res is not None
        out, yps = out_view(out and out[0], oshape, x) if act_pass else (None, None)
        yps = oshape[1] if out is None else yps
        if infer and spd:
            return _conv_infer_spd(x, g, wf, bias, spec, out, yps, f8)
        if infer:
            return _conv_infer(x, g, wf, bias, spec, res, rps, out, yps, f8)
        z, link = new_act(g.N, g.K, g.OH, g.OW, x), None
        if bn is None:
            _launch_conv_fwd(x, g, wf, bias, z, g.K, None, None, f8=f8)
            y = _act_pass(g, z, const_vec(g.K, 1.0, x.device), const_vec(g.K, 0.0, x.device), spec, res, rps, out, yps,
                          False, spd) if act_pass else z
            saved = (x, wt, z)
        else:
            stats = _conv_bn_stats(x, g, wf, bias, z, bn, train_bn, f8)
            saved = (x, wt, z, *stats, bn.weight)
            if (spec.defer and DEFER_AFFINE[0] and train_bn and need_grad and x.dtype == torch.bfloat16 and
                    spec.act == ACT_NONE and res is None and out is None and g.K % 8 == 0 and f8 is None and
                    g.groups == 1 and not spd):
                y, link = z, _defer_affine(z, stats, spec.act, g.K)
            else:
                y = _act_pass(g, z, stats[0], stats[1], spec, res, rps, out, yps, True, spd)
                if x.dtype == torch.bfloat16 and g.K % 128 == 0 and train_bn and not spd:
                    y._dmy_prod = spec
        _save_ctx(ctx, saved, g, spec, train_bn, link, weight, bias, gamma, beta, res is not None, xsink, rsink, spd)
        return y

    @staticmethod
    def backward(ctx, dy):
        g, spec = ctx.g, ctx.spec
        x, wt, z, *bnt = ctx.saved_tensors
        dy, dps = (vec_view if ctx.spd else pixel_stride)(dy.to(z.dtype))
        K, dev, dt = g.K, dy.device, dcode(dy)
        dbias = dgamma = dbeta = fused = None
        bias_in_wgrad = _dw_bias_in_wgrad(ctx)
        if spec.bn is not None:
            *stats, gamma = bnt
            *coef, dgamma, dbeta = _bn_bwd_coef(ctx, dt, dy, dps, z, stats, gamma)
            fused = None if ctx.spd else _bwd1x1(ctx, dy, dps, x, wt, z, stats, coef)
            if ctx.spd:
                dz, dzps = new_act(g.N, K, g.OH, g.OW, z), K
                call('dmy_bn_bwd_apply_s2d', dt, ptr(z), K, ptr(dy), dps, *map(ptr, stats), spec.act, *map(ptr, coef),
                     ptr(dz), K, g.N, g.OH, g.OW, K, stream())
            elif fused is None:
                dz, dzps = new_act(g.N, K, g.OH, g.OW, z), K
                call('dmy_bn_bwd_apply', dt, ptr(z), K, ptr(dy), dps, *map(ptr, stats), spec.act, *map(ptr, coef),
                     ptr(dz), K, g.M, K, stream())
            if ctx.has_bias and ctx.train_bn:
                dbias = _pgrad(ctx, 0, K, dev, zero=True)
        else:
            dz, dzps, dbias = _act_bias_bwd(ctx, dt, dy, dps, z, want_bias=not bias_in_wgrad)
        if fused is not None:
            dx, dw = fused
        else:
            dx = _dgrad(ctx, dt, dz, dzps, wt, z) if ctx.needs_input_grad[0] else None
            dw = None
            if ctx.needs_input_grad[1]:
                dw, db = _conv_wgrad(ctx, dt, x, dz, dzps, bias_in_wgrad)
                dbias = db if bias_in_wgrad else dbias
        dres = (dy if ctx.rsink is None else ctx.rsink.passthrough(dy)) if ctx.has_res else None
        return dx, dw, dbias, dgamma, dbeta, dres, None, None, None, None, None, None


def conv_bn_act(x, weight, bias, bn, stride, pad, act, res=None, spec=None, xsink=None, rsink=None, out=None,
                defer=False, spd=False):
    if spec is None:
        spec = _param_spec(weight._base if weight._base is not None else weight, stride, pad, act, bn)
    spec.defer = bool(defer)
    gamma = bn.weight if bn is not None else None
    beta = bn.bias if bn is not None else None
    return ConvBNActFn.apply(x, weight, bias, gamma, beta, res, spec, xsink, rsink, torch.is_grad_enabled(),
                             [out] if out is not None else None, bool(spd))



def _actbn_stats(z, g, spec, bn, train_bn):
    K, M, dev = g.K, g.M, z.device
    scale, shift = f32(K, dev), f32(K, dev)
    if not train_bn:
        call('dmy_bn_eval_coef', ptr(bn.weight), ptr(bn.bias), ptr(bn.running_mean), ptr(bn.running_var),
             float(bn.eps), K, ptr(scale), ptr(shift), stream())
        return scale, shift, const_vec(K, 0.0, dev), const_vec(K, 1.0, dev)
    mean, invstd = f32(K, dev), f32(K, dev)
    P = call('dmy_bn_partial_rows', M)
    psum, psq = f32(P * K, dev), f32(P * K, dev)
    call('dmy_actbn_stats', dcode(z), ptr(z), K, spec.act, M, K, ptr(psum), ptr(psq), stream())
    psum, psq, P = _fold_partials(psum, psq, P, K, dev)
    upd = int(bn.training and bn.track_running_stats)
    if upd:
        PARAM_GEN[0] += 1
    mom = bn.momentum if bn.momentum is not None else 0.0
    call('dmy_bn_finalize', ptr(psum), ptr(psq), P, K, float(M), ptr(bn.weight), ptr(bn.bias),
         ptr(bn.running_mean) if upd else None, ptr(bn.running_var) if upd else None,
         ptr(bn.num_batches_tracked) if upd else None, float(mom), float(bn.eps), upd,
         ptr(mean), ptr(invstd), ptr(scale), ptr(shift), stream())
    return scale, shift, mean, invstd


def _actbn_infer(x, g, wf, bias, spec, res, rps, y, yps):
    scale, shift = eval_coef(spec, x.device)
    dt = dcode(x)
    if g.groups != 1 and g.k != 9:
        z = new_act(g.N, g.K, g.OH, g.OW, x)
        _launch_conv_fwd(x, g, wf, bias, z, g.K, None, None)
        call('dmy_actbn_fwd', dt, ptr(z), g.K, spec.act, ptr(scale), ptr(shift), ptr(res), rps, ptr(y), yps, g.M, g.K,
             stream())
        return y
    if g.groups != 1:
        _dw_check(dt, x, wf, y, g, g.xps, yps)
        KernelTimer.run('dwconv_fwd', g.flops(), 'dmy_dwconv_fwd_actbn', dt, ptr(x), ptr(wf), ptr(bias), ptr(y), *g.dw(),
                        yps, ptr(scale), ptr(shift), spec.act, ptr(res), rps, stream(), tag=g.tag(),
                        nbytes=x.element_size() * (g.N * g.H * g.W * g.C + g.k * g.k * g.C + g.M * g.C))
        return y
    t = new_act(g.N, g.K, g.OH, g.OW, x)
    _launch_conv_fwd(x, g, wf, bias, t, g.K, None, None, epi=(None, None, spec.act, None, 0))
    call('dmy_actbn_fwd', dt, ptr(t), g.K, ACT_NONE, ptr(scale), ptr(shift), ptr(res), rps, ptr(y), yps, g.M, g.K, stream())
    return y


class ConvActBNFn(torch.autograd.Function):

    @staticmethod
    def forward(ctx, x, weight, bias, gamma, beta, res, spec, xsink=None, rsink=None, grad_on=True, out=None):
        need_grad = grad_on and any(ctx.needs_input_grad[:6])
        bn = spec.bn
        train_bn = bn.training or not bn.track_running_stats
        infer = not need_grad and not train_bn
        x, g, wf, wt, _ = _conv_operands(x, weight, spec, need_grad, infer)
        if g.K % VW[x.dtype] or g.s2d or g.Cp != g.C:
            raise NotImplementedError(f'conv -> act -> BN takes whole 16-byte vectors: output channels multiples of '
                                      f'{VW[x.dtype]} for {x.dtype}, got {g.K}')
        res, rps = vec_view(res) if res is not None else (None, 0)
        out, yps = out_view(out and out[0], (g.N, g.K, g.OH, g.OW), x)
        if out is not None and not vec_ok(x.dtype, (), [yps], [out]):
            out = None
        y = out if out is not None else new_act(g.N, g.K, g.OH, g.OW, x)
        yps = g.K if out is None else yps
        if infer:
            return _actbn_infer(x, g, wf, bias, spec, res, rps, y, yps)
        z = new_act(g.N, g.K, g.OH, g.OW, x)
        _launch_conv_fwd(x, g, wf, bias, z, g.K, None, None)
        scale, shift, mean, invstd = _actbn_stats(z, g, spec, bn, train_bn)
        call('dmy_actbn_fwd', dcode(z), ptr(z), g.K, spec.act, ptr(scale), ptr(shift), ptr(res), rps, ptr(y), yps, g.M,
             g.K, stream())
        _save_ctx(ctx, (x, wt, z, scale, mean, invstd), g, spec, train_bn, None, weight, bias, gamma, beta,
                  res is not None, xsink, rsink)
        return y

    @staticmethod
    def backward(ctx, dy):
        g, spec = ctx.g, ctx.spec
        x, wt, z, scale, mean, invstd = ctx.saved_tensors
        dy, dps = vec_view(dy.to(z.dtype))
        K, M, dev, dt = g.K, g.M, dy.device, dcode(dy)
        dbias = dgamma = dbeta = None
        P = call('dmy_bn_partial_rows', M)
        if ctx.train_bn:
            pdb, pdg = f32(P * K, dev), f32(P * K, dev)
            call('dmy_actbn_bwd_reduce', dt, ptr(z), K, ptr(dy), dps, ptr(mean), ptr(invstd), spec.act, M, K, ptr(pdb),
                 ptr(pdg), stream())
            pdb, pdg, R = _fold_partials(pdb, pdg, P, K, dev)
            ca, cb, cc = f32(K, dev), f32(K, dev), f32(K, dev)
            dgamma, dbeta = _pgrad(ctx, 1, K, dev), _pgrad(ctx, 2, K, dev)
            call('dmy_bn_bwd_finalize', ptr(pdb), ptr(pdg), R, K, float(M), ptr(spec.bn.weight), ptr(invstd), ptr(dgamma),
                 ptr(dbeta), ptr(ca), ptr(cb), ptr(cc), stream())
        else:
            ca, cb = scale, const_vec(K, 0.0, dev)
            cc = cb
        dz = new_act(g.N, K, g.OH, g.OW, z)
        pdz = f32(P * K, dev) if ctx.has_bias else None
        call('dmy_actbn_bwd_apply', dt, ptr(z), K, ptr(dy), dps, ptr(mean), ptr(invstd), spec.act, ptr(ca), ptr(cb),
             ptr(cc), ptr(dz), K, M, K, ptr(pdz), stream())
        if ctx.has_bias:
            dbias = _pgrad(ctx, 0, K, dev)
            call('dmy_reduce_rows', ptr(pdz), P, K, ptr(dbias), 0, stream())
        dx = _dgrad(ctx, dt, dz, K, wt, z) if ctx.needs_input_grad[0] else None
        dw = _conv_wgrad(ctx, dt, x, dz, K)[0] if ctx.needs_input_grad[1] else None
        dres = (dy if ctx.rsink is None else ctx.rsink.passthrough(dy)) if ctx.has_res else None
        return dx, dw, dbias, dgamma, dbeta, dres, None, None, None, None, None


def conv_act_bn(x, weight, bias, bn, stride, pad, act, res=None, spec=None, xsink=None, rsink=None, out=None):
    if spec is None:
        spec = _param_spec(weight._base if weight._base is not None else weight, stride, pad, act, bn)
    return ConvActBNFn.apply(x, weight, bias, bn.weight, bn.bias, res, spec, xsink, rsink, torch.is_grad_enabled(),
                             [out] if out is not None else None)



class MaxPoolFn(torch.autograd.Function):
    @staticmethod
    def forward(ctx, x, k, sink=None, out=None):
        x, xps = pixel_stride(x)
        N, C, H, W = x.shape
        y, yps = out_view(out and out[0], (N, C, H, W), x)
        if y is None:
            y, yps = new_act(N, C, H, W, x), C
        arg = torch.empty((N, H, W, C), dtype=torch.uint8, device=x.device)
        call('dmy_maxpool_fwd', dcode(x), ptr(x), xps, ptr(y), yps, ptr(arg), N, H, W, C, k, stream())
        ctx.save_for_backward(arg)
        ctx.k, ctx.shape, ctx.sink = k, (N, C, H, W), sink
        return y

    @staticmethod
    def backward(ctx, dy):
        (arg,) = ctx.saved_tensors
        N, C, H, W = ctx.shape
        dy, dps = pixel_stride(dy)
        buf, bps, acc = sink_target(ctx.sink, N, C, H, W, dy)
        call('dmy_maxpool_bwd', dcode(dy), ptr(dy), dps, ptr(arg), ptr(buf), bps, acc, N, H, W, C, ctx.k, stream())
        return sink_result(ctx.sink, buf), None, None, None


def maxpool_chain3(x, k, outs=(None, None, None)):
    if torch.is_grad_enabled() or k not in (3, 5) or x.dtype not in (torch.bfloat16, torch.float32):
        return None
    x, xps = pixel_stride(x)
    N, C, H, W = x.shape
    vw = VW[x.dtype]
    views = [out_view(o, (N, C, H, W), x) for o in outs]
    yps = views[0][1]
    if yps is not None and all(ps == yps for _, ps in views):
        ys = [v for v, _ in views]
    else:
        ys, yps = [new_act(N, C, H, W, x) for _ in range(3)], C
    if not vec_ok(x.dtype, [C], [xps, yps], [x] + ys) or N * (C // vw) >= 65536:
        return None
    call('dmy_maxpool_chain3_fwd', dcode(x), ptr(x), xps, ptr(ys[0]), ptr(ys[1]), ptr(ys[2]), yps, N, H, W, C, k,
# ... 959 lines not shown
```

### dma-yolo_amd/dmayolo/models/common.py

```python
import ctypes
import functools
import logging
import math
import os
import weakref
from copy import copy
from pathlib import Path

import numpy as np
import torch
import torch.nn as nn

from .. import functional as Fn
from ..functional import ACT_NONE, ACT_SILU, ACT_HARDSWISH, ACT_SIGMOID, ACT_GELU, ACT_RELU, ACT_LEAKY
from ..functional import call, ptr, stream
from ..utils.general import make_divisible, nms_padded, xyxy2xywh
from ..utils.torch_utils import time_sync

_LOG = logging.getLogger('dmayolo')

__all__ = ['autopad', 'Conv', 'DWConv', 'GhostConv', 'GhostBottleneck', 'C3Ghost', 'Bottleneck', 'C3', 'SPPF', 'SPPFCSPC', 'SCConv', 'CoorAttention', 'CA',
           'CABottleneck', 'C3CA', 'Concat', 'AdConcat2', 'AdConcat3', 'AdaptConcat', 'Adapt_Add2', 'Adapt_Add3', 'AdaptADD',
           'Upsample', 'C3STR', 'SwinTransformerBlock',
           'SwinTransformerLayer', 'WindowAttention', 'Mlp', 'DropPath', 'space_to_depth', 'SM', 'MP', 'DMConv', 'DMMConv',
# ... 27 lines not shown
        return ACT_LEAKY
    raise NotImplementedError(f'activation {type(m).__name__} has no gfx950 kernel')


def _pad_int(p):
    return p if isinstance(p, int) else p[0]


def conv_forward(conv, bn, act, x, res=None, xsink=None, rsink=None, out=None, defer=False):
    assert conv.dilation in (1, (1, 1)), 'dilated conv not on the DMA-YOLO path'
    s = conv.stride if isinstance(conv.stride, int) else conv.stride[0]
    pad, a = _pad_int(conv.padding), act_code(act)
    return Fn.conv_bn_act(x, conv.weight, conv.bias, bn, s, pad, a, res=res, spec=Fn.spec_for(conv, s, pad, a, bn),
                          xsink=xsink, rsink=rsink, out=out, defer=defer)


class Conv(nn.Module):

    def __init__(self, c1, c2, k=1, s=1, p=None, g=1, act=True):
        super().__init__()
        self.conv = nn.Conv2d(c1, c2, k, s, autopad(k, p), groups=g, bias=False)
        self.bn = nn.BatchNorm2d(c2)
        self.act = nn.SiLU() if act is True else (act if isinstance(act, nn.Module) else nn.Identity())

    def forward(self, x, res=None, xsink=None, rsink=None, out=None):
        return conv_forward(self.conv, self.bn, self.act, x, res, xsink, rsink, out)

    def forward_fuse(self, x, res=None, xsink=None, rsink=None, out=None):
        return conv_forward(self.conv, None, self.act, x, res, xsink, rsink, out)


class DWConv(Conv):

    def __init__(self, c1, c2, k=1, s=1, act=True):
        super().__init__(c1, c2, k, s, g=math.gcd(c1, c2), act=act)


class GhostConv(nn.Module):

    def __init__(self, c1, c2, k=1, s=1, g=1, act=True):
        super().__init__()
        c_ = c2 // 2
        self.cv1 = Conv(c1, c_, k, s, None, g, act)
        self.cv2 = Conv(c_, c_, 5, 1, None, c_, act)

    def forward(self, x, xsink=None):
        c_ = self.cv1.conv.out_channels
        c = self.cv1.conv
        OH, OW = Fn.conv_out_hw(x.shape[2], x.shape[3], c.kernel_size[0], c.stride[0], c.padding[0])
        cat = Fn.concat_buffer(x.shape[0], 2 * c_, OH, OW, x)
        sk = Fn.GradSink(2, adopt=False)
        y = self.cv1(x, xsink=xsink, out=cat[:, :c_])
        return Fn.ConcatFn.apply(None, 0.0, (sk, None), y, self.cv2(y, xsink=sk, out=cat[:, c_:]))


class GhostBottleneck(nn.Module):

    def __init__(self, c1, c2, k=3, s=1):
        super().__init__()
        c_ = c2 // 2
        self.conv = nn.Sequential(GhostConv(c1, c_, 1, 1),
                                  DWConv(c_, c_, k, s, act=False) if s == 2 else nn.Identity(),
                                  GhostConv(c_, c2, 1, 1, act=False))
        self.shortcut = nn.Sequential(DWConv(c1, c1, k, s, act=False),
                                      Conv(c1, c2, 1, 1, act=False)) if s == 2 else nn.Identity()

    def forward(self, x):
        sk = Fn.GradSink(2)
        a = self.conv[0](x, xsink=sk)
        if not isinstance(self.conv[1], nn.Identity):
            a = self.conv[1](a)
        a = self.conv[2](a)
        if isinstance(self.shortcut, nn.Identity):
            return Fn.AddFn.apply(x, a, sk)
        return Fn.AddFn.apply(self.shortcut[1](self.shortcut[0](x, xsink=sk)), a, None)


class Bottleneck(nn.Module):

    def __init__(self, c1, c2, shortcut=True, g=1, e=0.5):
        super().__init__()
        c_ = int(c2 * e)
        self.cv1 = Conv(c1, c_, 1, 1)
        self.cv2 = Conv(c_, c2, 3, 1, g=g)
        self.add = shortcut and c1 == c2

    def forward(self, x, out=None):
        if not self.add:
            return self.cv2(self.cv1(x), out=out)
        sk = Fn.GradSink(2)
        return self.cv2(self.cv1(x, xsink=sk), res=x, rsink=sk, out=out)


_INPLACE_CAT = int(os.environ.get('DMY_INPLACE_CAT', '2'))


_C3_PAIR = os.environ.get('DMY_C3_PAIR', '1') == '1'
_PAIRS = weakref.WeakKeyDictionary()


class _PairBN:
    training, track_running_stats, momentum = False, True, None

    def __init__(self, a, b):
        self.eps = a.eps
        self.weight, self.bias, self.running_mean, self.running_var = (
            torch.cat([getattr(a, n).detach(), getattr(b, n).detach()])
            for n in ('weight', 'bias', 'running_mean', 'running_var'))


class C3(nn.Module):

    def __init__(self, c1, c2, n=1, shortcut=True, g=1, e=0.5):
        super().__init__()
        c_ = int(c2 * e)
        self.cv1 = Conv(c1, c_, 1, 1)
        self.cv2 = Conv(c1, c_, 1, 1)
        self.cv3 = Conv(2 * c_, c2, 1)
        self.m = nn.Sequential(*(Bottleneck(c_, c_, shortcut, g, e=1.0) for _ in range(n)))

    def _pair(self):
        c1, c2 = self.cv1, self.cv2
        b1, b2 = getattr(c1, 'bn', None), getattr(c2, 'bn', None)
        w1, w2 = c1.conv.weight, c2.conv.weight
        if (b1 is None) != (b2 is None) or type(c1.act) is not type(c2.act) or w1.shape[1:] != w2.shape[1:] or \
                tuple(w1.shape[2:]) != (1, 1) or tuple(c1.conv.stride) != (1, 1) or tuple(c2.conv.stride) != (1, 1) or \
                (b1 is not None and (b1.eps != b2.eps or b1.training or b2.training)) or \
                (c1.conv.bias is None) != (c2.conv.bias is None):
            return None
        srcs = [w1, w2, c1.conv.bias, c2.conv.bias] + ([b1.weight, b1.bias, b1.running_mean, b1.running_var, b2.weight,
                                                        b2.bias, b2.running_mean, b2.running_var] if b1 is not None else [])
        key = (Fn.PARAM_GEN[0],) + tuple((t.data_ptr(), t._version) if t is not None else None for t in srcs)
        ent = _PAIRS.get(self)
        if ent is None or ent[0] != key:
            w = torch.cat([w1.detach(), w2.detach()])
            b = torch.cat([c1.conv.bias.detach(), c2.conv.bias.detach()]) if c1.conv.bias is not None else None
            ent = _PAIRS[self] = (key, w, b, _PairBN(b1, b2) if b1 is not None else None, act_code(c1.act))
        return ent[1:]

    def forward(self, x, out=None):
        blocks = list(self.m) if isinstance(self.m, nn.Sequential) else []
        seq = bool(blocks) and type(blocks[-1]) is Bottleneck and _INPLACE_CAT >= 1
        pair = self._pair() if seq and _C3_PAIR and not self.training and not torch.is_grad_enabled() else None
        if pair is not None:
            w, b, bn, act = pair
            c_ = w.shape[0] // 2
            cat = Fn.concat_buffer(x.shape[0], 2 * c_, x.shape[2], x.shape[3], x)
            Fn.conv_bn_act(x, w, b, bn, 1, 0, act, out=cat)
            a = cat[:, :c_]
            for blk in blocks[:-1]:
                a = blk(a)
            a = blocks[-1](a, out=cat[:, :c_])
            return self.cv3(Fn.ConcatFn.apply(None, 0.0, None, a, cat[:, c_:]), out=out)
        sk = Fn.GradSink(2)
        a = self.cv1(x, xsink=sk)
        if not seq and not (getattr(self.m, 'dmy_out', False) and _INPLACE_CAT >= 2):
            return self.cv3(Fn.ConcatFn.apply(None, 0.0, None, self.m(a), self.cv2(x, xsink=sk)), out=out)
        c_ = a.shape[1]
        cat = Fn.concat_buffer(a.shape[0], 2 * c_, a.shape[2], a.shape[3], a)
        if seq:
            for b in blocks[:-1]:
                a = b(a)
            a = blocks[-1](a, out=cat[:, :c_])
        else:
            a = self.m(a, out=cat[:, :c_])
        return self.cv3(Fn.ConcatFn.apply(None, 0.0, None, a, self.cv2(x, xsink=sk, out=cat[:, c_:])), out=out)


class C3Ghost(C3):

    def __init__(self, c1, c2, n=1, shortcut=True, g=1, e=0.5):
        super().__init__(c1, c2, n, shortcut, g, e)
        c_ = int(c2 * e)
        self.m = nn.Sequential(*(GhostBottleneck(c_, c_) for _ in range(n)))


class SPPF(nn.Module):

    def __init__(self, c1, c2, k=5):
        super().__init__()
        c_ = c1 // 2
        self.cv1 = Conv(c1, c_, 1, 1)
        self.cv2 = Conv(c_ * 4, c2, 1, 1)
        self.m = nn.MaxPool2d(kernel_size=k, stride=1, padding=k // 2)

    def forward(self, x):
        k = self.m.kernel_size
        c_ = self.cv1.conv.out_channels
        if _INPLACE_CAT >= 1:
            cat = Fn.concat_buffer(x.shape[0], 4 * c_, x.shape[2], x.shape[3], x)
            sl = [cat[:, i * c_:(i + 1) * c_] for i in range(4)]
        else:
            sl = [None] * 4
        x = self.cv1(x, out=sl[0])
        ys = Fn.maxpool_chain3(x, k, sl[1:])
        if ys is not None:
            return self.cv2(Fn.ConcatFn.apply(None, 0.0, None, x, *ys))
        s0, s1, s2 = Fn.GradSink(2), Fn.GradSink(2), Fn.GradSink(2)
        y1 = Fn.MaxPoolFn.apply(x, k, s0, sl[1:2])
        y2 = Fn.MaxPoolFn.apply(y1, k, s1, sl[2:3])
        return self.cv2(Fn.ConcatFn.apply(None, 0.0, (s0, s1, s2, None), x, y1, y2,
                                          Fn.MaxPoolFn.apply(y2, k, s2, sl[3:4])))


class SPPFCSPC(nn.Module):

    def __init__(self, c1, c2, n=1, shortcut=False, g=1, e=0.5, k=5):
        super().__init__()
        c_ = int(2 * c2 * e)
        self.cv1 = Conv(c1, c_, 1, 1)
        self.cv2 = Conv(c1, c_, 1, 1)
        self.cv3 = Conv(c_, c_, 3, 1)
        self.cv4 = Conv(c_, c_, 1, 1)
        self.m = nn.MaxPool2d(kernel_size=k, stride=1, padding=k // 2)
        self.cv5 = Conv(4 * c_, c_, 1, 1)
        self.cv6 = Conv(c_, c_, 3, 1)
        self.cv7 = Conv(2 * c_, c2, 1, 1)

    def forward(self, x):
        k = self.m.kernel_size
        c_ = self.cv1.conv.out_channels
        N, H, W = x.shape[0], x.shape[2], x.shape[3]
        if _INPLACE_CAT >= 1:
            cat = Fn.concat_buffer(N, 4 * c_, H, W, x)
            sl = [cat[:, i * c_:(i + 1) * c_] for i in range(4)]
            cat2 = Fn.concat_buffer(N, 2 * c_, H, W, x)
            s2l = [cat2[:, :c_], cat2[:, c_:]]
        else:
            sl, s2l = [None] * 4, [None] * 2
        sx = Fn.GradSink(2)
        x1 = self.cv4(self.cv3(self.cv1(x, xsink=sx)), out=sl[0])
        ys = Fn.maxpool_chain3(x1, k, sl[1:])
        if ys is not None:
            y1 = self.cv6(self.cv5(Fn.ConcatFn.apply(None, 0.0, None, x1, *ys)), out=s2l[0])
        else:
            s1, s2, s3 = Fn.GradSink(2), Fn.GradSink(2), Fn.GradSink(2)
            x2 = Fn.MaxPoolFn.apply(x1, k, s1, sl[1:2])
            x3 = Fn.MaxPoolFn.apply(x2, k, s2, sl[2:3])
            y1 = self.cv6(self.cv5(Fn.ConcatFn.apply(None, 0.0, (s1, s2, s3, None), x1, x2, x3,
                                                     Fn.MaxPoolFn.apply(x3, k, s3, sl[3:4]))), out=s2l[0])
        y2 = self.cv2(x, xsink=sx, out=s2l[1])
        return self.cv7(Fn.ConcatFn.apply(None, 0.0, None, y1, y2))


class SCConv(nn.Module):

    def __init__(self, c1, c2, stride, groups=1, dilation=1, pooling_r=4):
        super().__init__()
        self.k2 = nn.Sequential(nn.AvgPool2d(kernel_size=pooling_r, stride=pooling_r),
                                nn.Conv2d(c1, c1, 3, 1, autopad(3, None), dilation=dilation, groups=groups,
                                          bias=False),
                                nn.BatchNorm2d(c1))
        self.k3 = nn.Sequential(nn.Conv2d(c1, c1, 3, 1, autopad(3, None), dilation=dilation, groups=groups,
                                          bias=False),
                                nn.BatchNorm2d(c1))
        self.k4 = nn.Sequential(nn.Conv2d(c1, c2, 3, stride, autopad(3, None), dilation=dilation, groups=groups,
                                          bias=False),
                                nn.BatchNorm2d(c2))

    def forward(self, x, xsink=None):
        r = self.k2[0].kernel_size
        r = r if isinstance(r, int) else r[0]
        sk = Fn.GradSink(3) if xsink is None else xsink.expect(3)
        g = conv_forward(self.k2[1], self.k2[2], None, Fn.AvgPoolFn.apply(x, r, sk))
        u3 = conv_forward(self.k3[0], self.k3[1], None, x, xsink=sk, defer=True)
        return conv_forward(self.k4[0], self.k4[1], None, Fn.SCGateFn.apply(x, u3, g, sk))


class CoorAttention(nn.Module):

    def __init__(self, c1, c2, reduction=32):
        super().__init__()
        self.pool_h = nn.AdaptiveAvgPool2d((None, 1))
        self.pool_w = nn.AdaptiveAvgPool2d((1, None))
        c_ = max(8, c1 // reduction)
        self.conv1 = nn.Conv2d(c1, c_, kernel_size=1, stride=1, padding=0)
        self.bn1 = nn.BatchNorm2d(c_)
        self.act = nn.Hardswish()
        self.conv_w = nn.Conv2d(c_, c2, kernel_size=1, stride=1, padding=0)
        self.conv_h = nn.Conv2d(c_, c2, kernel_size=1, stride=1, padding=0)

    def forward(self, x):
        y = conv_forward(self.conv1, self.bn1, self.act, Fn.CAPoolFn.apply(x))
        lh = conv_forward(self.conv_h, None, None, y)
        lw = conv_forward(self.conv_w, None, None, y)
        return Fn.CAApplyFn.apply(x, lh, lw)


CA = CoorAttention


class CABottleneck(nn.Module):

    def __init__(self, c1, c2, shortcut=True, g=1, e=0.5, reduction=32):
        super().__init__()
        c_ = int(c2 * e)
        self.cv1 = Conv(c1, c_, 1, 1)
        self.cv2 = Conv(c_, c2, 3, 1, g=g)
        self.ca = CoorAttention(c2, c2, reduction)
        self.add = shortcut and c1 == c2

    def forward(self, x):
        if not self.add:
            return self.ca(self.cv2(self.cv1(x)))
        sk = Fn.GradSink(2)
        return Fn.AddFn.apply(x, self.ca(self.cv2(self.cv1(x, xsink=sk))), sk)


class C3CA(C3):
# ... 772 lines not shown
```

### include/dmayolo.h

```cpp
#ifndef DMAYOLO_H
#define DMAYOLO_H
#ifdef __cplusplus
extern "C" {
#endif

int dmy_conv_fwd_partial_rows(long M, int K);
long dmy_conv_fwd_bound_rows(long M, int K);
long dmy_conv_fwd_last_rows(void);
int dmy_conv_fwd_bn_rows(int dtype, const void* x, const void* w_ohwi, const float* bias, const void* y, int N,
                                int H, int W, int C, long xps, int K, int KH, int KW, int S, int P, int OH, int OW,
                                long yps);
int dmy_conv_fwd(int dtype, const void* x, const void* w_ohwi, const float* bias, void* y, float* psum, float* psq,
                 int N, int H, int W, int C, long xps, int K, int KH, int KW, int S, int P, int OH, int OW, long yps,
                 void* stream);
int dmy_conv_fwd_act(int dtype, const void* x, const void* w_ohwi, const float* bias, void* y, int N, int H, int W,
                     int C, long xps, int K, int KH, int KW, int S, int P, int OH, int OW, long yps, const float* scale,
                     const float* shift, int act, const void* res, long rps, void* stream);
long dmy_conv_fwd_splitk_elems(int dtype, const void* x, const void* w_ohwi, const void* y, int N, int H, int W, int C,
                               long xps, int K, int KH, int KW, int S, int P, int OH, int OW, long yps);
int dmy_conv_fwd_act_ws(int dtype, const void* x, const void* w_ohwi, const float* bias, void* y, int N, int H, int W,
                        int C, long xps, int K, int KH, int KW, int S, int P, int OH, int OW, long yps, const float* scale,
                        const float* shift, int act, const void* res, long rps, float* ws, long ws_elems, void* stream);
int dmy_conv_dgrad(int dtype, const void* dy, const void* w_ihwo, void* dx, int accumulate, int N, int H, int W, int C,
                   long xps, int K, int KH, int KW, int S, int P, int OH, int OW, long yps, void* stream);
int dmy_conv_wgrad(int dtype, const void* x, const void* dy, float* dw_ohwi, int N, int H, int W, int C, long xps,
                   int K, int KH, int KW, int S, int P, int OH, int OW, long yps, void* stream);
int dmy_conv1x1_bwd_bn_ok(long M, int K, int C, long dps, long xps, long bps, const void* dy, const void* z,
                          const void* x, const void* dx);
int dmy_conv1x1_bwd_bn(const void* dy, long dps, const void* z, const void* x, long xps, const void* wt,
                       const float* scale, const float* shift, const float* mean, const float* invstd, int act,
                       const float* ca, const float* cb, const float* cc, void* dx, long bps, int accumulate,
                       float* dw, float* ws, long ws_elems, long M, int K, int C, void* stream);
long dmy_conv1x1_bwd_bn_ws_elems(long M, int K, int C);
int dmy_conv_wgrad_ex(int dtype, const void* x, const void* dy, float* dw, int N, int H, int W, int C, long xps, int K,
                      int KH, int KW, int S, int P, int OH, int OW, long yps, int flags, void* stream);
long dmy_conv_wgrad_ws_elems(int dtype, const void* x, const void* dy, int N, int H, int W, int C, long xps, int K,
                             int KH, int KW, int S, int P, int OH, int OW, long yps, int flags);
int dmy_conv_wgrad_det(int dtype, const void* x, const void* dy, float* dw, int N, int H, int W, int C, long xps,
                       int K, int KH, int KW, int S, int P, int OH, int OW, long yps, int flags, float* ws,
                       long ws_elems, void* stream);
int dmy_conv_route(int pass, int dtype, const void* a, const void* b, const void* c, int N, int H, int W, int C,
                   long xps, int K, int KH, int KW, int S, int P, int OH, int OW, long yps, int acc);
enum {
  DMY_KERN_HALO = 0,
  DMY_KERN_SPLITK = 1,
  DMY_KERN_P1S = 2,
  DMY_KERN_STEM = 3,
  DMY_KERN_P1P = 4,
  DMY_KERN_PIPE8 = 5,
  DMY_KERN_WIDE = 6,
  DMY_KERN_WIDE288 = 7,
  DMY_KERN_TALL = 8,
  DMY_KERN_V3 = 9,
  DMY_KERN_V2 = 10,
  DMY_KERN_V2_BIG = 11,
  DMY_KERN_S2_Q2S = 12,
  DMY_KERN_S2_Q2 = 13,
  DMY_KERN_S2_MERGED = 14,
  DMY_KERN_S2_CLASS = 15,
  DMY_KERN_W_TAP128 = 16,
  DMY_KERN_W_TAP64 = 17,
  DMY_KERN_W_TAP64X2 = 18,
  DMY_KERN_W_V4 = 19,
  DMY_KERN_W_V3 = 20,
  DMY_KERN_W_V3N128 = 21,
  DMY_KERN_W_V3N256 = 22,
  DMY_KERN_W_V2_128 = 23,
  DMY_KERN_W_V2_64 = 24
};
int dmy_conv_wprep(int dtype, const float* w_oihw, void* w_ohwi, void* w_ihwo, int K, int C, int Cp, int KH, int KW,
                   void* stream);
int dmy_conv_wprep_multi(int dtype, const void* descs, int n, void* stream);
int dmy_conv_wprep_s2d(int dtype, const float* w_oihw, void* w_s2d, int K, int C, int Cs, void* stream);
int dmy_conv_wgrad_s2d_to_oihw(const float* dw_s2d, float* dw_oihw, int K, int C, int Cs, void* stream);
int dmy_conv_wgrad_to_oihw(const float* dw_ohwi, float* dw_oihw, int K, int C, int Cp, int KH, int KW, void* stream);

int dmy_dwconv_ok(int dtype, const void* x, const void* w, const void* z, int N, int H, int W, int C, int K, int groups,
                  long xps, int KH, int KW, int S, int P, int OH, int OW, long zps);
int dmy_dwconv_fwd_rows(long M, int C);
int dmy_dwconv_fwd(int dtype, const void* x, const void* w, const float* bias, void* z, float* psum, float* psq, int N,
                   int H, int W, int C, long xps, int KH, int KW, int S, int P, int OH, int OW, long zps, void* stream);
int dmy_dwconv_fwd_act(int dtype, const void* x, const void* w, const float* bias, void* y, int N, int H, int W, int C,
                       long xps, int KH, int KW, int S, int P, int OH, int OW, long yps, const float* scale,
                       const float* shift, int act, const void* res, long rps, void* stream);
int dmy_dwconv_dgrad(int dtype, const void* dz, const void* w, void* dx, int accumulate, int N, int H, int W, int C,
                     long xps, int KH, int KW, int S, int P, int OH, int OW, long zps, void* stream);
int dmy_dwconv_wgrad_rows(long M, int C);
int dmy_dwconv_wgrad(int dtype, const void* x, const void* dz, float* part, int N, int H, int W, int C, long xps, int KH,
                     int KW, int S, int P, int OH, int OW, long zps, void* stream);
int dmy_dwconv_wgrad_finalize(const float* part, int rows, int C, int KH, int KW, float* dw, int accumulate,
                              void* stream);
int dmy_dwconv_wgrad_bias(int dtype, const void* x, const void* dz, float* part, int N, int H, int W, int C, long xps,
                          int KH, int KW, int S, int P, int OH, int OW, long zps, void* stream);
int dmy_dwconv_wgrad_bias_finalize(const float* part, int rows, int C, int KH, int KW, float* dw, int accumulate,
                                   float* dbias, int bias_accumulate, void* stream);
int dmy_dwconv_fwd_actbn(int dtype, const void* x, const void* w, const float* bias, void* y, int N, int H, int W, int C,
                         long xps, int KH, int KW, int S, int P, int OH, int OW, long yps, const float* scale,
                         const float* shift, int act, const void* res, long rps, void* stream);

int dmy_actbn_stats(int dtype, const void* z, long zps, int act, long M, int C, float* psum, float* psq, void* stream);
int dmy_actbn_fwd(int dtype, const void* z, long zps, int act, const float* scale, const float* shift, const void* res,
                  long rps, void* y, long yps, long M, int C, void* stream);
int dmy_actbn_bwd_reduce(int dtype, const void* z, long zps, const void* dy, long dps, const float* mean,
                         const float* invstd, int act, long M, int C, float* pdb, float* pdg, void* stream);
int dmy_actbn_bwd_apply(int dtype, const void* z, long zps, const void* dy, long dps, const float* mean,
                        const float* invstd, int act, const float* ca, const float* cb, const float* cc, void* dz,
                        long dzps, long M, int C, float* pdz, void* stream);

int dmy_adapt_gate_blocks(int dtype, long M, int Ct, int L);
int dmy_adapt_gate_fwd(int dtype, int L, const void* x0, long x0ps, int C0, const void* x1, long x1ps, int C1,
                       const void* x2, long x2ps, int C2, const void* wm, long wmps, const float* W, const float* b,
                       void* y, long yps, float* a, long M, void* stream);
int dmy_adapt_gate_bwd(int dtype, int L, const void* dy, long dps, const void* x0, long x0ps, int C0, const void* x1,
                       long x1ps, int C1, const void* x2, long x2ps, int C2, const float* a, const void* wm, long wmps,
                       const float* W, void* dx0, long dx0ps, void* dx1, long dx1ps, void* dx2, long dx2ps,
                       int accumulate, void* dwm, long dwmps, float* pdw, float* pdb, long M, void* stream);
int dmy_adapt_add_fwd(int dtype, int n, const void* x0, long x0ps, const void* x1, long x1ps, const void* x2, long x2ps,
                      const float* w, float eps, void* y, long yps, long M, int C, void* stream);
int dmy_adapt_add_bwd(int dtype, int n, const void* dy, long dps, const void* x0, long x0ps, const void* x1, long x1ps,
                      const void* x2, long x2ps, const float* w, float eps, void* dx0, long dx0ps, void* dx1, long dx1ps,
                      void* dx2, long dx2ps, int accumulate, float* part, long M, int C, void* stream);

long dmy_fp8_quant_ws_elems(void);
int dmy_fp8_quant(const void* x_bf16, long rows, int C, long xps, void* x8, float* ws, void* stream);
int dmy_conv_wprep_fp8(const float* w_oihw, void* w8_ohwi, float* wscale, int K, int C, int KH, int KW, void* stream);
int dmy_conv_fwd_fp8_partial_rows(long M, int K);
int dmy_conv_fwd_fp8(const void* x8, const void* w8_ohwi, const float* xamax, const float* wscale, const float* bias,
                     void* y, float* psum, float* psq, int N, int H, int W, int C, int K, int KH, int KW, int S, int P,
                     int OH, int OW, long yps, const float* scale, const float* shift, int act, const void* res,
                     long rps, void* stream);

int dmy_bn_partial_rows(long M);
int dmy_bn_stats(int dtype, const void* z, long zps, long M, int C, float* psum, float* psq, void* stream);
int dmy_bn_finalize(const float* psum, const float* psq, int P, int C, double count, const float* gamma,
                    const float* beta, float* running_mean, float* running_var, long long* num_batches_tracked,
                    float momentum, float eps, int update, float* mean, float* invstd, float* scale, float* shift,
                    void* stream);
int dmy_bn_eval_coef(const float* gamma, const float* beta, const float* running_mean, const float* running_var,
                     float eps, int C, float* scale, float* shift, void* stream);
int dmy_bn_act_fwd(int dtype, const void* z, long zps, const float* scale, const float* shift, int act,
                   const void* res, long rps, void* y, long yps, long M, int C, void* stream);
int dmy_bn_act_f8_blocks(void);
int dmy_bn_act_fwd_f8(const void* z, long zps, const float* scale, const float* shift, int act, const void* res,
                      long rps, void* y, long yps, long M, int C, void* y8, const float* pmax, float* nmax, float* used,
                      float headroom, float* nsat, void* stream);
int dmy_bn_bwd_reduce(int dtype, const void* z, long zps, const void* dy, long dps, const float* scale,
                      const float* shift, const float* mean, const float* invstd, int act, long M, int C, float* pdb,
                      float* pdg, void* stream);
int dmy_bn_bwd_finalize(const float* pdb, const float* pdg, int P, int C, double count, const float* gamma,
                        const float* invstd, float* dgamma, float* dbeta, float* ca, float* cb, float* cc,
                        void* stream);
int dmy_bn_bwd_apply(int dtype, const void* z, long zps, const void* dy, long dps, const float* scale,
                     const float* shift, const float* mean, const float* invstd, int act, const float* ca,
                     const float* cb, const float* cc, void* dz, long dzps, long M, int C, void* stream);
int dmy_reduce_rows(const float* part, int P, int C, float* out, int accumulate, void* stream);
int dmy_bn_reduce_rows(int dtype, const void* z, long zps, const void* dy, long dps, long M, int C);
int dmy_colsum2_rows(long P);
int dmy_colsum2(const float* a, const float* b, long P, int C, float* oa, float* ob, void* stream);

int dmy_bn_act_s2d_fwd(int dtype, const void* z, long zps, const float* scale, const float* shift, int act, void* y,
                       long yps, int N, int H, int W, int K, void* stream);
int dmy_bn_bwd_reduce_s2d_rows(int dtype, long M, int K);
int dmy_bn_bwd_reduce_s2d(int dtype, const void* z, long zps, const void* dy, long dps, const float* scale,
                          const float* shift, const float* mean, const float* invstd, int act, int N, int H, int W,
                          int K, float* pdb, float* pdg, void* stream);
int dmy_bn_bwd_apply_s2d(int dtype, const void* z, long zps, const void* dy, long dps, const float* scale,
                         const float* shift, const float* mean, const float* invstd, int act, const float* ca,
                         const float* cb, const float* cc, void* dz, long dzps, int N, int H, int W, int K,
                         void* stream);
int dmy_maxpool2_fwd(int dtype, const void* x, long xps, void* y, long yps, unsigned char* argmax, int N, int H, int W,
                     int C, void* stream);
int dmy_maxpool2_bwd(int dtype, const void* dy, long dps, const unsigned char* argmax, void* dx, long dxps,
                     int accumulate, int N, int H, int W, int C, void* stream);
int dmy_spd_split_fwd(int dtype, const void* x, long xps, void* sm, long smps, void* mp, long mpps,
                      unsigned char* argmax, int N, int H, int W, int C, void* stream);
int dmy_spd_split_bwd(int dtype, const void* dsm, long dsmps, const void* dmp, long dmpps, const unsigned char* argmax,
                      void* dx, long dxps, int N, int H, int W, int C, void* stream);

int dmy_gate_fwd(int dtype, const void* a, long aps, const void* b, long bps, void* y, long yps, long M, int C,
                 float scale, void* stream);
int dmy_gate_bwd(int dtype, const void* dy, long dps, const void* a, long aps, const void* b, long bps, void* da,
                 long daps, void* db, long dbps, long M, int C, float scale, void* stream);
int dmy_layerscale_fwd(int dtype, const void* x, long xps, const void* y, const float* gamma, void* out, long ops,
                       long M, int C, void* stream);
int dmy_layerscale_bwd_rows(long M);
int dmy_layerscale_bwd(int dtype, const void* dout, long dps, const void* y, const float* gamma, void* dy, long M,
                       int C, float* part, void* stream);

int dmy_maxpool_fwd(int dtype, const void* x, long xps, void* y, long yps, unsigned char* argmax, int N, int H, int W,
                    int C, int k, void* stream);
int dmy_maxpool_bwd(int dtype, const void* dy, long dps, const unsigned char* argmax, void* dx, long dxps,
                    int accumulate, int N, int H, int W, int C, int k, void* stream);
int dmy_maxpool_chain3_fwd(int dtype, const void* x, long xps, void* y1, void* y2, void* y3, long yps, int N, int H,
                           int W, int C, int k, void* stream);
int dmy_avgpool_fwd(int dtype, const void* x, long xps, void* y, int N, int H, int W, int C, int r, void* stream);
int dmy_avgpool_bwd(int dtype, const void* dy, void* dx, long dxps, int accumulate, int N, int H, int W, int C, int r,
                    void* stream);
int dmy_resize_fwd(int dtype, const void* x, long xps, void* y, long yps, float yscale, int N, int IH, int IW, int OH,
                   int OW, int C, void* stream);
int dmy_resize_bwd(int dtype, const void* dy, long dps, void* dx, long dxps, int N, int IH, int IW, int OH, int OW,
                   int C, void* stream);
int dmy_slice_copy(int dtype, const void* src, long sps, void* dst, long dps, long M, int C, const float* w, int idx,
                   int nw, float eps, int accumulate, void* stream);
int dmy_dot_partial_blocks(long M, int C);
int dmy_dot_partial(int dtype, const void* a, long aps, const void* b, long bps, long M, int C, float* part,
                    void* stream);
int dmy_slice_copy_dot(int dtype, const void* dy, long dps, void* g, long gps, const void* x, long xps, long M, int C,
                       const float* wv, int idx, int nw, float eps, int accumulate, float* part, void* stream);
int dmy_bifpn_wgrad(const float* part, int nblk, int nw, const float* w, float eps, float* dw, void* stream);
int dmy_scgate_fwd(int dtype, const void* x, long xps, const void* u3, const void* g, void* out, int N, int H, int W,
                   int C, int GH, int GW, void* stream);
int dmy_scgate_bwd(int dtype, const void* x, long xps, const void* u3, const void* g, const void* dout, void* du3,
                   void* dpre, long dpps, int accumulate, int N, int H, int W, int C, int GH, int GW, void* stream);
int dmy_scgate_bn_rows(int N, int H, int W, int C);
int dmy_scgate_bn_fwd(const void* x, long xps, const void* z, const float* scale, const float* shift, const void* g,
                      void* out, int N, int H, int W, int C, int GH, int GW, void* stream);
int dmy_scgate_bn_bwd(const void* x, long xps, const void* z, const float* scale, const float* shift,
                      const float* mean, const float* invstd, const void* g, const void* dout, void* du3, void* dpre,
                      int N, int H, int W, int C, int GH, int GW, float* pdb, float* pdg, void* stream);
int dmy_ca_pool_fwd(int dtype, const void* x, long xps, void* y, int N, int H, int W, int C, void* stream);
int dmy_ca_pool_bwd(int dtype, const void* dy, void* dx, long dxps, int accumulate, int N, int H, int W, int C,
                    void* stream);
int dmy_ca_apply_fwd(int dtype, const void* x, long xps, const void* lh, const void* lw, void* out, long ops, int N,
                     int H, int W, int C, void* stream);
int dmy_ca_apply_bwd(int dtype, const void* x, long xps, const void* lh, const void* lw, const void* dout, long dps,
                     void* dx, long dxps, void* dlh, void* dlw, int N, int H, int W, int C, void* stream);
int dmy_image_s2d(int dtype, int src_kind, const void* x, void* y, int N, int C, int H, int W, int Cs, float scale,
                  void* stream);
int dmy_nchw_to_nhwc(int dtype, int src_kind, const void* x, void* y, int N, int C, int H, int W, int Cp, float scale,
                     void* stream);
int dmy_tta_image(int dtype, int src_kind, const void* x, void* y, int N, int C, int H, int W, int s2d, int Cs,
                  float scale, int flip, int OH, int OW, int OHp, int OWp, float pad_value, void* stream);
int dmy_nhwc_to_nchw_f32(int dtype, const void* x, long xps, float* y, int N, int C, int H, int W, void* stream);
int dmy_pointwise(int dtype, int op, int act, const void* a, const void* b, void* y, long n, float alpha,
                  void* stream);
int dmy_cast(int src_kind, int dst_kind, const void* x, void* y, long n, float scale, void* stream);

int dmy_detect_decode(int dtype, const void* y, long sb, long sh, long sw, int N, int H, int W, int na, int no,
                      float stride, const float* anchors, float* z, long zoff, long ztotal, void* stream);
int dmy_detect_decode_levels(int dtype, int nl, const void* const* ys, const long* strides, const int* hw,
                             const float* lvl_stride, int N, int na, int no, const float* anchors, float* z, long ztotal,
                             void* stream);
int dmy_detect_decode_tta(int dtype, int nl, const void* const* ys, const long* strides, const int* hw,
                          const float* lvl_stride, int N, int na, int no, const float* anchors, float* z, long ztotal,
                          float scale, int flip, float img_h, float img_w, int level_mask, long zoff, void* stream);
int dmy_build_targets(const float* targets, int nt, const float* anchors, int na, int H, int W, float anchor_t,
                      int* b, int* a, int* gj, int* gi, int* tcls, float* tbox, float* anch, int* count,
                      void* stream);
int dmy_yolo_loss_part_rows(void);
int dmy_yolo_loss_level(int dtype, const void* p, long sb, long sa, long sh, long sw, int N, int na, int H, int W,
                        int no, int nc, float box_gain, float obj_gain, float cls_gain, float cls_pw, float obj_pw,
                        float cp, float cn, float balance, float bs, const int* b, const int* a, const int* gj,
                        const int* gi, const int* tcls, const float* tbox, const float* anch, const int* count,
                        int cap, float* grad, float* tobj, float* part, float* tgrad, int* links, void* stream);
int dmy_yolo_loss_finalize(const float* part, int nl, float box, float obj, float cls, float bs, float* loss,
                           float* items, void* stream);
int dmy_yolo_loss_level_focal(int dtype, const void* p, long sb, long sa, long sh, long sw, int N, int na, int H, int W,
                              int no, int nc, float box_gain, float obj_gain, float cls_gain, float cls_pw,
                              float obj_pw, float cp, float cn, const double* balance, int level, float fl_gamma,
                              float bs, const int* b, const int* a, const int* gj, const int* gi, const int* tcls,
                              const float* tbox, const float* anch, const int* count, int cap, float* grad,
                              float* tobj, float* part, float* tgrad, int* links, void* stream);
int dmy_yolo_loss_finalize_balance(const float* part, int nl, float box, float obj, float cls, float bs,
                                   double* balance, int autobalance, int ssi, float* loss, float* items,
                                   void* stream);
int dmy_loss_grad(int dtype, const float* grad, const float* upstream, void* dp, long n, void* stream);
int dmy_siou_eval(const float* b1, const float* b2, float* iou, float* grad_b1, int n, void* stream);

int dmy_nms_candidates(const float* pred, int nimg, int A, int no, float conf, int multi_label,
                       const unsigned char* class_ok, unsigned long long* keys, long cap, int* counts, void* stream);
int dmy_nms_sort(unsigned long long* keys, long cap, const int* counts, int nimg, void* stream);
int dmy_nms_greedy(const float* pred, int nimg, int A, int no, float iou, int agnostic, int max_det, int max_nms,
                   const unsigned long long* keys, long cap, int* counts, float* boxes, float* out, int* nkeep,
                   int* ncand, void* stream);
int dmy_nms_mask_rows(void);
int dmy_nms_greedy_mask(const float* pred, int nimg, int A, int no, float iou, int agnostic, int max_det, int max_nms,
                        const unsigned long long* keys, long cap, int* counts, float* boxes,
                        unsigned long long* mask, float* out, int* nkeep, int* ncand, void* stream);

int dmy_layernorm_fwd(int dtype, const void* x, long xps, const float* w, const float* b, void* y, float* mean,
                      float* rstd, long M, int C, float eps, void* stream);
int dmy_layernorm_bwd_blocks(long M);
int dmy_layernorm_bwd(int dtype, const void* x, long xps, const void* dy, long dps, const float* w, const float* mean,
                      const float* rstd, void* dx, long dxps, int accumulate, long M, int C, float* pdw, float* pdb,
                      void* stream);
int dmy_winattn_fwd(int dtype, const void* qkv, const float* table, void* out, int B, int H, int W, int C, int nh,
                    int shift, float scale, void* stream);
int dmy_winattn_bwd_groups(int B, int H, int W, int nh);
int dmy_winattn_bwd(int dtype, const void* qkv, const void* dout, const float* table, void* dqkv, float* dtab_part,
                    float* dtab, int B, int H, int W, int C, int nh, int shift, float scale, void* stream);
int dmy_sample_scale(int dtype, const void* x, const float* scale, void* y, long per, long n, void* stream);
int dmy_droppath_add(int dtype, const void* x, const void* f, const float* u, float keep, void* y, long per, long n,
                     void* stream);
int dmy_droppath_grad(int dtype, const void* dy, const float* u, float keep, void* df, long per, long n, void* stream);

int dmy_chunk_size(void);
int dmy_sgd(float* const* p, const float* const* g, float* const* m, const long* n, const int* tid, const long* off,
            int nchunks, float lr, float momentum, float weight_decay, int nesterov, const float* scale,
            const float* found, void* stream);
int dmy_adam(float* const* p, const float* const* g, float* const* m, float* const* v, const long* n, const int* tid,
             const long* off, int nchunks, float lr, float beta1, float beta2, float eps, float weight_decay,
             float bias_corr1, float bias_corr2_sqrt, const float* scale, const float* found, int* dstep,
             void* stream);
int dmy_amp_check(const float* const* g, const long* n, const int* tid, const long* off, int nchunks,
                  const float* scale, float* found, void* stream);
int dmy_amp_update(float* scale, float* gup, int* tracker, float* found, float world, float growth, float backoff,
                   int interval, void* stream);
// ... 68 lines not shown
```

Baseline: 165.3 images/s.

## Fuse C3 cv1/cv2 1x1 convs into one stacked conv with dual-output BN kernels

After: 163.6 images/s. 1.0% lower.

```diff
diff --git a/dma-yolo_amd/csrc/bn.hip b/dma-yolo_amd/csrc/bn.hip
--- a/dma-yolo_amd/csrc/bn.hip
+++ b/dma-yolo_amd/csrc/bn.hip
@@ -29,7 +29,7 @@
   }
 }
 
-__global__ void bn_finalize_kernel(const float* __restrict__ psum, const float* __restrict__ psq, int P, int C,
+__global__ void bn_finalize_kernel(const float* __restrict__ psum, const float* __restrict__ psq, int P, int ld,
                                    double count, const float* __restrict__ gamma, const float* __restrict__ beta,
                                    float* __restrict__ rmean, float* __restrict__ rvar, long long* nbt, float momentum,
                                    float eps, int update, float* __restrict__ mean, float* __restrict__ invstd,
@@ -39,8 +39,8 @@
   double a = 0.0, b = 0.0;
 #pragma unroll 8
   for (int p = threadIdx.x; p < P; p += blockDim.x) {
-    a += (double)psum[(long)p * C + c];
-    b += (double)psq[(long)p * C + c];
+    a += (double)psum[(long)p * ld + c];
+    b += (double)psq[(long)p * ld + c];
   }
   sa[threadIdx.x] = a;
   sb[threadIdx.x] = b;
@@ -134,6 +134,32 @@
   }
 }
 
+template <typename T>
+__global__ void __launch_bounds__(256) bn_act_fwd2_vec(const T* __restrict__ z, long zps, const float* __restrict__ scale,
+                                                       const float* __restrict__ shift, int act, T* __restrict__ y0,
+                                                       long y0ps, T* __restrict__ y1, long y1ps, int csplit, long M,
+                                                       int C, int rev) {
+  constexpr int VW = Traits<T>::VW;
+  RowMap rm(C, VW);
+  if (!rm.active()) return;
+  const int c0 = rm.cv * VW;
+  float sc[VW], sh[VW];
+  ldf<VW>(scale + c0, sc);
+  ldf<VW>(shift + c0, sh);
+  T* __restrict__ y = c0 < csplit ? y0 + c0 : y1 + (c0 - csplit);
+  const long yps = c0 < csplit ? y0ps : y1ps;
+  const long S = (long)gridDim.x * rm.RB;
+  for (long m = (long)blockIdx.x * rm.RB + rm.rr; m < M; m += S) {
+    const long mu = rev ? M - 1 - m : m;
+    float f[VW];
+    unpack<T>(*reinterpret_cast<const uint4*>(z + mu * zps + c0), f);
+#pragma unroll
+    for (int j = 0; j < VW; ++j) f[j] = f[j] * sc[j] + sh[j];
+    act_fwd_n<VW>(act, f);
+    *reinterpret_cast<uint4*>(y + mu * yps) = pack<T>(f);
+  }
+}
+
 __global__ void __launch_bounds__(256) bn_act_fwd_f8_kernel(const bf16* __restrict__ z, long zps,
                                                             const float* __restrict__ scale,
                                                             const float* __restrict__ shift, int act,
@@ -218,7 +244,8 @@
 
 template <typename T, bool STATS, int U = 1>
 __global__ void __launch_bounds__(256) bn_bwd_reduce_vec(const T* __restrict__ z, long zps, const T* __restrict__ dy,
-                                                         long dps, const float* __restrict__ scale,
+                                                         long dps, const T* __restrict__ dy1, long dps1, int csplit,
+                                                         const float* __restrict__ scale,
                                                          const float* __restrict__ shift, const float* __restrict__ mean,
                                                          const float* __restrict__ invstd, int act, long M, int C,
                                                          float* __restrict__ pdb, float* __restrict__ pdg, int rev) {
@@ -245,6 +272,8 @@
       ldf<VW>(mean + c0, mu);
       ldf<VW>(invstd + c0, is);
     }
+    const T* __restrict__ dyc = c0 < csplit ? dy + c0 : dy1 + (c0 - csplit);
+    const long dpc = c0 < csplit ? dps : dps1;
     const long S = (long)gridDim.x * rm.RB;
     for (long m = (long)blockIdx.x * rm.RB + rm.rr; m < M; m += S * U) {
       uint4 zv[U], gv[U];
@@ -253,7 +282,7 @@
         const long mu = rev ? M - 1 - (m + u * S) : m + u * S;
         if (m + u * S < M) {
           zv[u] = *reinterpret_cast<const uint4*>(z + mu * zps + c0);
-          if (!STATS) gv[u] = *reinterpret_cast<const uint4*>(dy + mu * dps + c0);
+          if (!STATS) gv[u] = *reinterpret_cast<const uint4*>(dyc + mu * dpc);
         }
       }
 #pragma unroll
@@ -402,7 +431,7 @@
   }
 }
 
-__global__ void bn_bwd_finalize_kernel(const float* __restrict__ pdb, const float* __restrict__ pdg, int P, int C,
+__global__ void bn_bwd_finalize_kernel(const float* __restrict__ pdb, const float* __restrict__ pdg, int P, int ld,
                                        double count, const float* __restrict__ gamma, const float* __restrict__ invstd,
                                        float* __restrict__ dgamma, float* __restrict__ dbeta, float* __restrict__ ca,
                                        float* __restrict__ cb, float* __restrict__ cc) {
@@ -411,8 +440,8 @@
   double a = 0.0, b = 0.0;
 #pragma unroll 8
   for (int p = threadIdx.x; p < P; p += blockDim.x) {
-    a += (double)pdb[(long)p * C + c];
-    b += (double)pdg[(long)p * C + c];
+    a += (double)pdb[(long)p * ld + c];
+    b += (double)pdg[(long)p * ld + c];
   }
   sa[threadIdx.x] = a;
   sb[threadIdx.x] = b;
@@ -476,7 +505,7 @@
     hipStream_t st = (hipStream_t)stream;
     if (vec_ok(VW, C, {zps}, {}, {z}) && C / VW <= 256) {
       bn_bwd_reduce_vec<T, true><<<row_grid(M, C, VW, kRedCap), 256, 0, st>>>(
-          (const T*)z, zps, (const T*)z, zps, nullptr, nullptr, nullptr, nullptr, 0, M, C, psum, psq, 0);
+          (const T*)z, zps, (const T*)z, zps, nullptr, 0, C, nullptr, nullptr, nullptr, nullptr, 0, M, C, psum, psq, 0);
     } else {
       const int P = dmy_bn_partial_rows(M);
       const int rpb = (int)((M + P - 1) / P);
@@ -489,7 +518,16 @@
 DMY_API int dmy_bn_finalize(const float* psum, const float* psq, int P, int C, double count, const float* gamma,
                             const float* beta, float* rmean, float* rvar, long long* nbt, float momentum, float eps,
                             int update, float* mean, float* invstd, float* scale, float* shift, void* stream) {
-  bn_finalize_kernel<<<C, 256, 0, (hipStream_t)stream>>>(psum, psq, P, C, count, gamma, beta, rmean, rvar, nbt,
+  return dmy_bn_finalize_ld(psum, psq, P, C, C, count, gamma, beta, rmean, rvar, nbt, momentum, eps, update, mean, invstd,
+                            scale, shift, stream);
+}
+
+DMY_API int dmy_bn_finalize_ld(const float* psum, const float* psq, int P, int C, int ld, double count,
+                               const float* gamma, const float* beta, float* rmean, float* rvar, long long* nbt,
+                               float momentum, float eps, int update, float* mean, float* invstd, float* scale,
+                               float* shift, void* stream) {
+  if (ld < C) return kInvalid;
+  bn_finalize_kernel<<<C, 256, 0, (hipStream_t)stream>>>(psum, psq, P, ld, count, gamma, beta, rmean, rvar, nbt,
                                                          momentum, eps, update, mean, invstd, scale, shift);
   return (int)hipGetLastError();
 }
@@ -517,6 +555,20 @@
   });
 }
 
+DMY_API int dmy_bn_act_fwd2(int dtype, const void* z, long zps, const float* scale, const float* shift, int act,
+                            void* y0, long y0ps, void* y1, long y1ps, int csplit, long M, int C, void* stream) {
+  return by_dtype(dtype, kInvalid, [&](auto tag) {
+    using T = typename decltype(tag)::type;
+    constexpr int VW = Traits<T>::VW;
+    if (csplit <= 0 || csplit >= C || csplit % VW || C / VW > 256 || y0ps < csplit || y1ps < C - csplit || zps < C ||
+        !vec_ok(VW, C, {zps, y0ps, y1ps}, {z, y0, y1}))
+      return kInvalid;
+    bn_act_fwd2_vec<T><<<row_grid(M, C, VW, kEwCap), 256, 0, (hipStream_t)stream>>>(
+        (const T*)z, zps, scale, shift, act, (T*)y0, y0ps, (T*)y1, y1ps, csplit, M, C, kRevAct);
+    return (int)hipGetLastError();
+  });
+}
+
 DMY_API int dmy_bn_act_f8_blocks(void) { return 1024; }
 
 DMY_API int dmy_bn_act_fwd_f8(const void* z, long zps, const float* scale, const float* shift, int act, const void* res,
@@ -546,13 +598,29 @@
     hipStream_t st = (hipStream_t)stream;
     if (vec_ok(VW, C, {zps, dps}, {}, {z, dy}) && C / VW <= 256) {
       bn_bwd_reduce_vec<T, false><<<row_grid(M, C, VW, kRedCap), 256, 0, st>>>(
-          (const T*)z, zps, (const T*)dy, dps, scale, shift, mean, invstd, act, M, C, pdb, pdg, kRevReduce);
+          (const T*)z, zps, (const T*)dy, dps, nullptr, 0, C, scale, shift, mean, invstd, act, M, C, pdb, pdg, kRevReduce);
     } else {
       const int P = dmy_bn_partial_rows(M);
       const int rpb = (int)((M + P - 1) / P);
       bn_bwd_reduce_kernel<T><<<dim3(P, ceil_div(C, 64)), 256, 0, st>>>((const T*)z, zps, (const T*)dy, dps, scale, shift,
                                                                         mean, invstd, act, M, C, rpb, pdb, pdg);
     }
+    return (int)hipGetLastError();
+  });
+}
+
+DMY_API int dmy_bn_bwd_reduce2(int dtype, const void* z, long zps, const void* dy0, long dps0, const void* dy1,
+                               long dps1, int csplit, const float* scale, const float* shift, const float* mean,
+                               const float* invstd, int act, long M, int C, float* pdb, float* pdg, void* stream) {
+  return by_dtype(dtype, kInvalid, [&](auto tag) {
+    using T = typename decltype(tag)::type;
+    constexpr int VW = Traits<T>::VW;
+    if (csplit <= 0 || csplit >= C || csplit % VW || C / VW > 256 || dps0 < csplit || dps1 < C - csplit || zps < C ||
+        !vec_ok(VW, C, {zps, dps0, dps1}, {z, dy0, dy1}))
+      return kInvalid;
+    bn_bwd_reduce_vec<T, false><<<row_grid(M, C, VW, kRedCap), 256, 0, (hipStream_t)stream>>>(
+        (const T*)z, zps, (const T*)dy0, dps0, (const T*)dy1, dps1, csplit, scale, shift, mean, invstd, act, M, C, pdb,
+        pdg, kRevReduce);
     return (int)hipGetLastError();
   });
 }
@@ -570,7 +638,14 @@
 DMY_API int dmy_bn_bwd_finalize(const float* pdb, const float* pdg, int P, int C, double count, const float* gamma,
                                 const float* invstd, float* dgamma, float* dbeta, float* ca, float* cb, float* cc,
                                 void* stream) {
-  bn_bwd_finalize_kernel<<<C, 256, 0, (hipStream_t)stream>>>(pdb, pdg, P, C, count, gamma, invstd, dgamma, dbeta, ca,
+  return dmy_bn_bwd_finalize_ld(pdb, pdg, P, C, C, count, gamma, invstd, dgamma, dbeta, ca, cb, cc, stream);
+}
+
+DMY_API int dmy_bn_bwd_finalize_ld(const float* pdb, const float* pdg, int P, int C, int ld, double count,
+                                   const float* gamma, const float* invstd, float* dgamma, float* dbeta, float* ca,
+                                   float* cb, float* cc, void* stream) {
+  if (ld < C) return kInvalid;
+  bn_bwd_finalize_kernel<<<C, 256, 0, (hipStream_t)stream>>>(pdb, pdg, P, ld, count, gamma, invstd, dgamma, dbeta, ca,
                                                              cb, cc);
   return (int)hipGetLastError();
 }
diff --git a/dma-yolo_amd/csrc/bwd1x1.hip b/dma-yolo_amd/csrc/bwd1x1.hip
--- a/dma-yolo_amd/csrc/bwd1x1.hip
+++ b/dma-yolo_amd/csrc/bwd1x1.hip
@@ -56,14 +56,16 @@
   static_assert(LDS <= 160 * 1024, "LDS");
 };
 
-template <int K, int CB, int TP, int PX>
+template <int K, int CB, int TP, int PX, bool DUAL>
 __global__ void __launch_bounds__(256, 1) conv1x1_bwd_bn(
-    const bf16* __restrict__ dy, long dps, const bf16* __restrict__ z, const bf16* __restrict__ x, long xps,
-    const bf16* __restrict__ wt, const float* __restrict__ scale, const float* __restrict__ shift,
+    const bf16* __restrict__ dy, long dps, const bf16* __restrict__ dy1, long dps1, int ksplit,
+    const bf16* __restrict__ z, long zps, const bf16* __restrict__ x, long xps,
+    const bf16* __restrict__ wt, const bf16* __restrict__ wt1, const float* __restrict__ scale,
+    const float* __restrict__ shift,
     const float* __restrict__ mean, const float* __restrict__ invstd, int act, const float* __restrict__ ca,
     const float* __restrict__ cb, const float* __restrict__ cc, bf16* __restrict__ dx, long bps, int accumulate,
-    float* __restrict__ dw, float* __restrict__ dws, long M, int ntiles, int C, int nsplit, unsigned dyb, unsigned zb,
-    unsigned xb) {
+    float* __restrict__ dw, float* __restrict__ dw1, float* __restrict__ dws, long M, int ntiles, int C, int nsplit,
+    unsigned dyb, unsigned zb, unsigned xb) {
   using S = Shape<K, CB, TP, PX>;
   extern __shared__ __attribute__((aligned(16))) char b1_smem[];
   bf16* ws = reinterpret_cast<bf16*>(b1_smem);
@@ -76,11 +78,15 @@
   x += cbase;
   dx += cbase;
   dw += cbase;
+  if (DUAL) dw1 += cbase;
 
   for (int e = tid; e < CB * S::KCH; e += S::NT) {
     const int r = e / S::KCH, ch = e % S::KCH;
-    *reinterpret_cast<uint4*>(ws + r * K + (wsw<K>(r, ch) << 3)) =
-        *reinterpret_cast<const uint4*>(wt + (long)(cbase + r) * K + ch * 8);
+    const bf16* src = wt + (long)(cbase + r) * K + ch * 8;
+    if (DUAL)
+      src = ch * 8 < ksplit ? wt + (long)(cbase + r) * ksplit + ch * 8
+                            : wt1 + (long)(cbase + r) * (K - ksplit) + (ch * 8 - ksplit);
+    *reinterpret_cast<uint4*>(ws + r * K + (wsw<K>(r, ch) << 3)) = *reinterpret_cast<const uint4*>(src);
   }
 
   const int kc8 = (tid % S::KCH) * 8, xc8 = (tid % S::CCH) * 8;
@@ -102,6 +108,8 @@
   }
 
   const __amdgpu_buffer_rsrc_t rdy = rsrc(dy, dyb), rz = rsrc(z, zb), rx = rsrc(x, xb - 2u * cbase);
+  const bf16* dyp = (DUAL && kc8 >= ksplit) ? dy1 + (kc8 - ksplit) : dy + kc8;
+  const long dpp = (DUAL && kc8 >= ksplit) ? dps1 : dps;
   uint4 pg[S::NDZ], pz[S::NDZ], pxv[S::NX];
   auto issue = [&](int t) {
     const long m0 = (long)t * TP;
@@ -109,8 +117,9 @@
     for (int j = 0; j < S::NDZ; ++j) {
       const long m = m0 + tid / S::KCH + j * S::RDZ;
       const bool ok = m < M;
-      pg[j] = bload(rdy, ok ? (unsigned)((m * dps + kc8) * 2) : kOob);
-      pz[j] = bload(rz, ok ? (unsigned)((m * K + kc8) * 2) : kOob);
+      if (DUAL) pg[j] = *reinterpret_cast<const uint4*>(dyp + (ok ? m : M - 1) * dpp);
+      else pg[j] = bload(rdy, ok ? (unsigned)((m * dps + kc8) * 2) : kOob);
+      pz[j] = bload(rz, ok ? (unsigned)((m * zps + kc8) * 2) : kOob);
     }
 #pragma unroll
     for (int j = 0; j < S::NX; ++j) {
@@ -244,19 +253,22 @@
       for (int r = 0; r < 4; ++r) {
         const int kk = wk * S::KW + i * 16 + 4 * g + r, c = wc * S::CW + j * 16 + il;
         if (part != nullptr) part[kk * CB + c] = wacc[i][j][r];
+        else if (DUAL && kk >= ksplit) atomicAdd(dw1 + (long)(kk - ksplit) * C + c, wacc[i][j][r]);
         else atomicAdd(dw + (long)kk * C + c, wacc[i][j][r]);
       }
 }
 
-__global__ void __launch_bounds__(256) wgrad_slots_reduce(const float* __restrict__ dws, float* __restrict__ dw, int K,
-                                                          int C, int CB, int nblocks, int nsplit) {
+__global__ void __launch_bounds__(256) wgrad_slots_reduce(const float* __restrict__ dws, float* __restrict__ dw,
+                                                          float* __restrict__ dw1, int ksplit, int K, int C, int CB,
+                                                          int nblocks, int nsplit) {
   const long e = (long)blockIdx.x * blockDim.x + threadIdx.x;
   if (e >= (long)K * C) return;
   const int k = (int)(e / C), c = (int)(e % C), cs = c / CB, cl = c % CB;
   float s = 0.f;
   for (int b = 0; b < nblocks; ++b)
     if (((b >> 3) % nsplit) == cs) s += dws[((long)b * K + k) * CB + cl];
-  dw[e] += s;
+  if (k < ksplit) dw[e] += s;
+  else dw1[(long)(k - ksplit) * C + c] += s;
 }
 
 int num_cus() {
@@ -288,55 +300,40 @@
   return ngrp * ns;
 }
 
-template <int K, int C>
-int launch(const bf16* dy, long dps, const bf16* z, const bf16* x, long xps, const bf16* wt, const float* scale,
-           const float* shift, const float* mean, const float* invstd, int act, const float* ca, const float* cb,
-           const float* cc, bf16* dx, long bps, int acc, float* dw, float* ws, long M, hipStream_t st) {
+struct Args {
+  const bf16 *dy, *dy1, *z, *x, *wt, *wt1;
+  long dps, dps1, zps, xps, bps, M;
+  const float *scale, *shift, *mean, *invstd, *ca, *cb, *cc;
+  bf16* dx;
+  float *dw, *dw1, *ws;
+  int ksplit, act, acc;
+};
+
+template <int K, int C, bool DUAL>
+int launch(const Args& a, hipStream_t st) {
   constexpr Plan pl = plan(K, C);
   constexpr int CB = pl.cb, TP = pl.tp, PX = pl.px, NS = C / CB;
   using S = Shape<K, CB, TP, PX>;
   static bool raised = false;
   if (!raised) {
-    (void)hipFuncSetAttribute((const void*)conv1x1_bwd_bn<K, CB, TP, PX>,
+    (void)hipFuncSetAttribute((const void*)conv1x1_bwd_bn<K, CB, TP, PX, DUAL>,
                               hipFuncAttributeMaxDynamicSharedMemorySize, S::LDS);
     raised = true;
   }
-  const int nb = grid_blocks(M, K, C);
-  conv1x1_bwd_bn<K, CB, TP, PX><<<nb, 256, S::LDS, st>>>(
-      dy, dps, z, x, xps, wt, scale, shift, mean, invstd, act, ca, cb, cc, dx, bps, acc, dw, ws, M, ceil_div(M, TP), C,
-      NS, (unsigned)(2.0 * (double)M * dps), (unsigned)(2.0 * (double)M * K), (unsigned)(2.0 * (double)M * xps));
-  if (ws != nullptr)
-    wgrad_slots_reduce<<<ceil_div((long)K * C, 256), 256, 0, st>>>(ws, dw, K, C, CB, nb, NS);
+  const int nb = grid_blocks(a.M, K, C);
+  const double M2 = 2.0 * (double)a.M;
+  conv1x1_bwd_bn<K, CB, TP, PX, DUAL><<<nb, 256, S::LDS, st>>>(
+      a.dy, a.dps, a.dy1, a.dps1, a.ksplit, a.z, a.zps, a.x, a.xps, a.wt, a.wt1, a.scale, a.shift, a.mean, a.invstd,
+      a.act, a.ca, a.cb, a.cc, a.dx, a.bps, a.acc, a.dw, a.dw1, a.ws, a.M, ceil_div(a.M, TP), C, NS,
+      DUAL ? 0u : (unsigned)(M2 * a.dps), (unsigned)(M2 * a.zps), (unsigned)(M2 * a.xps));
+  if (a.ws != nullptr)
+    wgrad_slots_reduce<<<ceil_div((long)K * C, 256), 256, 0, st>>>(a.ws, a.dw, a.dw1, a.ksplit, K, C, CB, nb, NS);
   return (int)hipGetLastError();
 }
-}
-}
-
-DMY_API int dmy_conv1x1_bwd_bn_ok(long M, int K, int C, long dps, long xps, long bps, const void* dy, const void* z,
-                                  const void* x, const void* dx) {
-  if (b1::plan(K, C).cb == 0 || M <= 0) return 0;
-  if (!vec_ok(8, 0, {dps, xps, bps}, {}, {dy, z, x, dx}) || dps < K || xps < C || bps < C) return 0;
-  const double lim = (double)b1::kOob - 64.0;
-  if (2.0 * (double)M * dps >= lim || 2.0 * (double)M * K >= lim || 2.0 * (double)M * xps >= lim) return 0;
-  return 1;
-}
-
-DMY_API long dmy_conv1x1_bwd_bn_ws_elems(long M, int K, int C) {
-  if (b1::plan(K, C).cb == 0 || M <= 0) return 0;
-  return (long)b1::grid_blocks(M, K, C) * K * b1::plan(K, C).cb;
-}
-
-DMY_API int dmy_conv1x1_bwd_bn(const void* dy, long dps, const void* z, const void* x, long xps, const void* wt,
-                               const float* scale, const float* shift, const float* mean, const float* invstd, int act,
-                               const float* ca, const float* cb, const float* cc, void* dx, long bps, int accumulate,
-                               float* dw, float* ws, long ws_elems, long M, int K, int C, void* stream) {
-  if (!dmy_conv1x1_bwd_bn_ok(M, K, C, dps, xps, bps, dy, z, x, dx)) return -1;
-  if (ws != nullptr && ws_elems < dmy_conv1x1_bwd_bn_ws_elems(M, K, C)) return -1;
-  hipStream_t st = (hipStream_t)stream;
-#define B1_GO(K_, C_)                                                                                                 \
-  if (K == K_ && C == C_)                                                                                            \
-    return b1::launch<K_, C_>((const bf16*)dy, dps, (const bf16*)z, (const bf16*)x, xps, (const bf16*)wt, scale,     \
-                              shift, mean, invstd, act, ca, cb, cc, (bf16*)dx, bps, accumulate, dw, ws, M, st);
+
+int go(int K, int C, const Args& a, hipStream_t st) {
+#define B1_GO(K_, C_) \
+  if (K == K_ && C == C_) return a.ksplit < K ? launch<K_, C_, true>(a, st) : launch<K_, C_, false>(a, st);
   B1_GO(64, 64)
   B1_GO(128, 64)
   B1_GO(64, 128)
@@ -349,3 +346,52 @@
 #undef B1_GO
   return -1;
 }
+}
+}
+
+DMY_API int dmy_conv1x1_bwd_bn2_ok(long M, int K, int C, int ksplit, long dps, long dps1, long zps, long xps, long bps,
+                                   const void* dy, const void* dy1, const void* z, const void* x, const void* dx) {
+  if (b1::plan(K, C).cb == 0 || M <= 0) return 0;
+  const bool dual = ksplit != K;
+  if (dual && (ksplit * 2 != K || !dy1)) return 0;
+  if (!vec_ok(8, ksplit, {dps, dual ? dps1 : 0, zps, xps, bps}, {dy, z, x, dx}, {dy1})) return 0;
+  if (dps < ksplit || (dual && dps1 < K - ksplit) || zps < K || xps < C || bps < C) return 0;
+  const double lim = (double)b1::kOob - 64.0;
+  if ((!dual && 2.0 * (double)M * dps >= lim) || 2.0 * (double)M * zps >= lim || 2.0 * (double)M * xps >= lim) return 0;
+  return 1;
+}
+
+DMY_API int dmy_conv1x1_bwd_bn_ok(long M, int K, int C, long dps, long xps, long bps, const void* dy, const void* z,
+                                  const void* x, const void* dx) {
+  return dmy_conv1x1_bwd_bn2_ok(M, K, C, K, dps, 0, K, xps, bps, dy, nullptr, z, x, dx);
+}
+
+DMY_API long dmy_conv1x1_bwd_bn_ws_elems(long M, int K, int C) {
+  if (b1::plan(K, C).cb == 0 || M <= 0) return 0;
+  return (long)b1::grid_blocks(M, K, C) * K * b1::plan(K, C).cb;
+}
+
+DMY_API int dmy_conv1x1_bwd_bn2(const void* dy, long dps, const void* dy1, long dps1, int ksplit, const void* z,
+                                long zps, const void* x, long xps, const void* wt, const void* wt1,
+                                const float* scale, const float* shift, const float* mean, const float* invstd, int act,
+                                const float* ca, const float* cb, const float* cc, void* dx, long bps, int accumulate,
+                                float* dw, float* dw1, float* ws, long ws_elems, long M, int K, int C, void* stream) {
+  if (!dmy_conv1x1_bwd_bn2_ok(M, K, C, ksplit, dps, dps1, zps, xps, bps, dy, dy1, z, x, dx)) return -1;
+  if (ksplit != K && (!wt1 || !dw1 || !al16(wt1))) return -1;
+  if (ws != nullptr && ws_elems < dmy_conv1x1_bwd_bn_ws_elems(M, K, C)) return -1;
+  b1::Args a;
+  a.dy = (const bf16*)dy, a.dy1 = (const bf16*)dy1, a.z = (const bf16*)z, a.x = (const bf16*)x;
+  a.wt = (const bf16*)wt, a.wt1 = (const bf16*)wt1;
+  a.dps = dps, a.dps1 = dps1, a.zps = zps, a.xps = xps, a.bps = bps, a.M = M;
+  a.scale = scale, a.shift = shift, a.mean = mean, a.invstd = invstd, a.ca = ca, a.cb = cb, a.cc = cc;
+  a.dx = (bf16*)dx, a.dw = dw, a.dw1 = dw1, a.ws = ws, a.ksplit = ksplit, a.act = act, a.acc = accumulate;
+  return b1::go(K, C, a, (hipStream_t)stream);
+}
+
+DMY_API int dmy_conv1x1_bwd_bn(const void* dy, long dps, const void* z, const void* x, long xps, const void* wt,
+                               const float* scale, const float* shift, const float* mean, const float* invstd, int act,
+                               const float* ca, const float* cb, const float* cc, void* dx, long bps, int accumulate,
+                               float* dw, float* ws, long ws_elems, long M, int K, int C, void* stream) {
+  return dmy_conv1x1_bwd_bn2(dy, dps, nullptr, 0, K, z, K, x, xps, wt, nullptr, scale, shift, mean, invstd, act, ca, cb,
+                             cc, dx, bps, accumulate, dw, nullptr, ws, ws_elems, M, K, C, stream);
+}
diff --git a/dma-yolo_amd/dmayolo/_lib.py b/dma-yolo_amd/dmayolo/_lib.py
--- a/dma-yolo_amd/dmayolo/_lib.py
+++ b/dma-yolo_amd/dmayolo/_lib.py
@@ -53,6 +53,8 @@
     'dmy_conv1x1_bwd_bn_ok': [L, I, I, L, L, L, P, P, P, P],
     'dmy_conv1x1_bwd_bn': [P, L, P, P, L, P, P, P, P, P, I, P, P, P, P, L, I, P, P, L, L, I, I, P],
     'dmy_conv1x1_bwd_bn_ws_elems': [L, I, I],
+    'dmy_conv1x1_bwd_bn2_ok': [L, I, I, I, L, L, L, L, L, P, P, P, P, P],
+    'dmy_conv1x1_bwd_bn2': [P, L, P, L, I, P, L, P, L, P, P, P, P, P, P, I, P, P, P, P, L, I, P, P, P, L, L, I, I, P],
     'dmy_aug_desc_bytes': [],
     'dmy_augment_batch': [P, I, P, I, I, P],
     'dmy_mosaic_desc_bytes': [],
@@ -76,6 +78,10 @@
     'dmy_bn_bwd_reduce': [I, P, L, P, L, P, P, P, P, I, L, I, P, P, P],
     'dmy_bn_bwd_finalize': [P, P, I, I, D, P, P, P, P, P, P, P, P],
     'dmy_bn_bwd_apply': [I, P, L, P, L, P, P, P, P, I, P, P, P, P, L, L, I, P],
+    'dmy_bn_finalize_ld': [P, P, I, I, I, D, P, P, P, P, P, F, F, I, P, P, P, P, P],
+    'dmy_bn_bwd_finalize_ld': [P, P, I, I, I, D, P, P, P, P, P, P, P, P],
+    'dmy_bn_act_fwd2': [I, P, L, P, P, I, P, L, P, L, I, L, I, P],
+    'dmy_bn_bwd_reduce2': [I, P, L, P, L, P, L, I, P, P, P, P, I, L, I, P, P, P],
     'dmy_reduce_rows': [P, I, I, P, I, P],
     'dmy_bn_reduce_rows': [I, P, L, P, L, L, I],
     'dmy_colsum2_rows': [L],
diff --git a/dma-yolo_amd/dmayolo/functional.py b/dma-yolo_amd/dmayolo/functional.py
--- a/dma-yolo_amd/dmayolo/functional.py
+++ b/dma-yolo_amd/dmayolo/functional.py
@@ -191,15 +191,16 @@
     def __init__(self, weights, dtype, dev):
         import numpy as np
         sizes = [-(-w.numel() // self.ALIGN) * self.ALIGN for w in weights]
-        self.buf = torch.empty(2 * sum(sizes), dtype=dtype, device=dev)
+        total = sum(sizes)
+        self.buf = torch.empty(2 * total, dtype=dtype, device=dev)
         self.map, recs, off = {}, [], 0
         for w, n in zip(weights, sizes):
             K, C, KH, KW = w.shape
             wf = self.buf[off:off + w.numel()].view(K, KH * KW * C)
-            wt = self.buf[off + n:off + n + w.numel()].view(C, KH * KW * K)
+            wt = self.buf[total + off:total + off + w.numel()].view(C, KH * KW * K)
             self.map[w.data_ptr()] = (wf, wt)
             recs.append((w.data_ptr(), wf.data_ptr(), wt.data_ptr(), K, C, KH, KW))
-            off += 2 * n
+            off += n
         rec = np.dtype([('w', '<u8'), ('wf', '<u8'), ('wt', '<u8'), ('K', '<i4'), ('C', '<i4'), ('KH', '<i4'),
                         ('KW', '<i4')])
         self.table = torch.from_numpy(np.array(recs, dtype=rec).view(np.uint8)).to(dev)
@@ -211,6 +212,15 @@
 
     def get(self, weight, dtype):
         return self.map.get(weight.data_ptr()) if dtype == self.dtype else None
+
+    def pair(self, w1, w2, dtype):
+        a, b = self.get(w1, dtype), self.get(w2, dtype)
+        if a is None or b is None or a[0].shape[1] != b[0].shape[1] or \
+                b[0].data_ptr() != a[0].data_ptr() + a[0].numel() * a[0].element_size():
+            return None
+        off = (a[0].data_ptr() - self.buf.data_ptr()) // self.buf.element_size()
+        n = a[0].numel() + b[0].numel()
+        return self.buf[off:off + n].view(a[0].shape[0] + b[0].shape[0], a[0].shape[1]), a[1], b[1]
 
 
 class ConvSpec:
@@ -908,6 +918,171 @@
 
 
 
+C3_PAIR_TRAIN = [os.environ.get('DMY_C3_PAIR_TRAIN', '1') == '1']
+C3_PAIR_BWD = [os.environ.get('DMY_C3_PAIR_BWD', 'auto')]
+
+
+def pair_stacked_bwd(K, C):
+    if C3_PAIR_BWD[0] in ('0', '1'):
+        return C3_PAIR_BWD[0] == '1'
+    return K <= 128
+
+
+def conv_pair_ok(x, conv1, bn1, act1, conv2, bn2, act2):
+    if not (C3_PAIR_TRAIN[0] and torch.is_grad_enabled() and bn1 is not None and bn2 is not None and x.dim() == 4):
+        return False
+    w1, w2 = conv1.weight, conv2.weight
+    if not (bn1.training and bn2.training and bn1.eps == bn2.eps and
+            bn1.track_running_stats == bn2.track_running_stats and act1 == act2):
+        return False
+    for c in (conv1, conv2):
+        if not (tuple(c.kernel_size) == (1, 1) and tuple(c.stride) == (1, 1) and _pad0(c.padding) and c.groups == 1 and
+                c.bias is None and c.dilation in (1, (1, 1)) and not getattr(c, 'dmy_fp8', False)):
+            return False
+    sp1, sp2 = _SPECS.get(conv1), _SPECS.get(conv2)
+    if (sp1 is not None and sp1.f8_emit is not None) or (sp2 is not None and sp2.f8_emit is not None):
+        return False
+    c_, C = w1.shape[0], w1.shape[1]
+    vw = VW.get(x.dtype)
+    return bool(vw and w1.shape == w2.shape and x.shape[1] == C and c_ % vw == 0 and C % vw == 0 and 2 * c_ // vw <= 256
+                and not getattr(x, '_dmy_s2d', 0) and x.requires_grad and w1.requires_grad and w2.requires_grad and
+                all(t.requires_grad for t in (bn1.weight, bn1.bias, bn2.weight, bn2.bias)))
+
+
+def _pad0(p):
+    return p in (0, (0, 0))
+
+
+def _pair_weights(w1, w2, dtype):
+    pre = WeightPrep.current.pair(w1, w2, dtype) if WeightPrep.current is not None else None
+    if pre is not None:
+        return pre
+    c_, C = w1.shape[0], w1.shape[1]
+    wf = torch.empty((2 * c_, C), dtype=dtype, device=w1.device)
+    wts = []
+    for h, w in enumerate((w1, w2)):
+        wt = torch.empty((C, c_), dtype=dtype, device=w1.device)
+        call('dmy_conv_wprep', DT[dtype], ptr(w.detach().contiguous()), ptr(wf[h * c_:]), ptr(wt), c_, C, C, 1, 1,
+             stream())
+        wts.append(wt)
+    return wf, wts[0], wts[1]
+
+
+class ConvPairFn(torch.autograd.Function):
+
+    @staticmethod
+    def forward(ctx, x, w1, w2, g1, b1, g2, b2, specs, out2=None):
+        bns = (specs[0].bn, specs[1].bn)
+        x, xps = pixel_stride(x)
+        N, C, H, W = x.shape
+        c_, dev, dt = w1.shape[0], x.device, dcode(x)
+        K, M = 2 * c_, N * H * W
+        g = ConvGeom(N, C, H, W, xps, K, 1, 1, 0, H, W, M, C, H, W, 1, 1, 0, C, 0)
+        wf, wt1, wt2 = _pair_weights(w1, w2, x.dtype)
+        z = new_act(N, K, H, W, x)
+        P = call('dmy_conv_fwd_bound_rows', M, K)
+        psum, psq = f32(P * K, dev), f32(P * K, dev)
+        _launch_conv_fwd(x, g, wf, None, z, K, psum, psq)
+        P = call('dmy_conv_fwd_last_rows')
+        psum, psq, P = _fold_partials(psum, psq, P, K, dev)
+        scale, shift, mean, invstd = f32(K, dev), f32(K, dev), f32(K, dev), f32(K, dev)
+        for h, bn in enumerate(bns):
+            o = h * c_
+            upd = int(bn.track_running_stats)
+            if upd:
+                PARAM_GEN[0] += 1
+            mom = bn.momentum if bn.momentum is not None else 0.0
+            call('dmy_bn_finalize_ld', ptr(psum[o:]), ptr(psq[o:]), P, c_, K, float(M), ptr(bn.weight), ptr(bn.bias),
+                 ptr(bn.running_mean) if upd else None, ptr(bn.running_var) if upd else None,
+                 ptr(bn.num_batches_tracked) if upd else None, float(mom), float(bn.eps), upd, ptr(mean[o:]),
+                 ptr(invstd[o:]), ptr(scale[o:]), ptr(shift[o:]), stream())
+        y1 = new_act(N, c_, H, W, x)
+        y2, y2ps = out_view(out2 and out2[0], (N, c_, H, W), x)
+        if y2 is None or not vec_ok(x.dtype, (), [y2ps], [y2]):
+            y2, y2ps = new_act(N, c_, H, W, x), c_
+        act = specs[0].act
+        call('dmy_bn_act_fwd2', dt, ptr(z), K, ptr(scale), ptr(shift), act, ptr(y1), c_, ptr(y2), y2ps, c_, M, K,
+             stream())
+        if x.dtype == torch.bfloat16 and c_ % 128 == 0:
+            y1._dmy_prod, y2._dmy_prod = specs
+        ctx.save_for_backward(x, wt1, wt2, z, scale, shift, mean, invstd, g1, g2)
+        ctx.g, ctx.act, ctx.arena = g, act, WgradArena.current
+        ctx.keys = tuple((w.data_ptr(), gm.data_ptr(), bt.data_ptr()) for w, gm, bt in ((w1, g1, b1), (w2, g2, b2)))
+        return y1, y2
+
+    @staticmethod
+    def _take(ctx, key, shape, dev, zero):
+        t = ctx.arena.take(key, shape) if ctx.arena is not None else None
+        if t is not None:
+            return t
+        return torch.zeros(shape, dtype=torch.float32, device=dev) if zero else \
+            torch.empty(shape, dtype=torch.float32, device=dev)
+
+    @staticmethod
+    def backward(ctx, dy1, dy2):
+        x, wt1, wt2, z, scale, shift, mean, invstd, gm1, gm2 = ctx.saved_tensors
+        g, act = ctx.g, ctx.act
+        N, C, H, W, xps, K, M = g.N, g.C, g.H, g.W, g.xps, g.K, g.M
+        c_, dev, dt, es = K // 2, z.device, dcode(z), z.element_size()
+        dys = [vec_view(d.to(z.dtype)) for d in (dy1, dy2)]
+        (d1, dps1), (d2, dps2) = dys
+        P = call('dmy_bn_reduce_rows', dt, ptr(z), K, ptr(d1), dps1, M, K)
+        pdb, pdg = f32(P * K, dev), f32(P * K, dev)
+        call('dmy_bn_bwd_reduce2', dt, ptr(z), K, ptr(d1), dps1, ptr(d2), dps2, c_, ptr(scale), ptr(shift), ptr(mean),
+             ptr(invstd), act, M, K, ptr(pdb), ptr(pdg), stream())
+        pdb, pdg, P = _fold_partials(pdb, pdg, P, K, dev)
+        ca, cb, cc = f32(K, dev), f32(K, dev), f32(K, dev)
+        pg, dws = [], []
+        for h, gm in enumerate((gm1, gm2)):
+            o, (wk, gk, bk) = h * c_, ctx.keys[h]
+            dgamma, dbeta = ConvPairFn._take(ctx, gk, (c_,), dev, False), ConvPairFn._take(ctx, bk, (c_,), dev, False)
+            call('dmy_bn_bwd_finalize_ld', ptr(pdb[o:]), ptr(pdg[o:]), P, c_, K, float(M), ptr(gm), ptr(invstd[o:]),
+                 ptr(dgamma), ptr(dbeta), ptr(ca[o:]), ptr(cb[o:]), ptr(cc[o:]), stream())
+            pg += [dgamma, dbeta]
+            dws.append(ConvPairFn._take(ctx, wk, (c_, C, 1, 1), dev, True))
+        dx = new_act(N, C, H, W, z)
+        stats, coef, wts = (scale, shift, mean, invstd), (ca, cb, cc), (wt1, wt2)
+        fused = BWD1X1[0] and z.dtype == torch.bfloat16
+        if fused and pair_stacked_bwd(K, C) and call(
+                'dmy_conv1x1_bwd_bn2_ok', M, K, C, c_, dps1, dps2, K, xps, C, ptr(d1), ptr(d2), ptr(z), ptr(x), ptr(dx)):
+            ne = call('dmy_conv1x1_bwd_bn_ws_elems', M, K, C) if DETERMINISTIC[0] else 0
+            ws = f32(ne, dev) if ne else None
+            KernelTimer.run('conv_bwd1x1', 4.0 * M * K * C, 'dmy_conv1x1_bwd_bn2', ptr(d1), dps1, ptr(d2), dps2, c_,
+                            ptr(z), K, ptr(x), xps, ptr(wt1), ptr(wt2), *map(ptr, stats), act, *map(ptr, coef), ptr(dx),
+                            C, 0, ptr(dws[0]), ptr(dws[1]), ptr(ws), ne, M, K, C, stream(), tag=g.tag(),
+                            nbytes=es * (2 * M * K + 2 * M * C + K * C) + 4 * K * C)
+            return (dx, dws[0], dws[1], *pg, None, None)
+        gh = g._replace(K=c_)
+        for h, (d, dps) in enumerate(dys):
+            o = h * c_
+            zh = z[:, o:o + c_]
+            st, co = [t[o:] for t in stats], [t[o:] for t in coef]
+            if fused and call('dmy_conv1x1_bwd_bn2_ok', M, c_, C, c_, dps, 0, K, xps, C, ptr(d), None, ptr(zh), ptr(x),
+                              ptr(dx)):
+                ne = call('dmy_conv1x1_bwd_bn_ws_elems', M, c_, C) if DETERMINISTIC[0] else 0
+                ws = f32(ne, dev) if ne else None
+                KernelTimer.run('conv_bwd1x1', 4.0 * M * c_ * C, 'dmy_conv1x1_bwd_bn2', ptr(d), dps, None, 0, c_,
+                                ptr(zh), K, ptr(x), xps, ptr(wts[h]), None, *map(ptr, st), act, *map(ptr, co), ptr(dx),
+                                C, h, ptr(dws[h]), None, ptr(ws), ne, M, c_, C, stream(), tag=gh.tag(),
+                                nbytes=es * (2 * M * c_ + (2 + h) * M * C + c_ * C) + 4 * c_ * C)
+                continue
+            dz = new_act(N, c_, H, W, z)
+            call('dmy_bn_bwd_apply', dt, ptr(zh), K, ptr(d), dps, *map(ptr, st), act, *map(ptr, co), ptr(dz), c_, M,
+                 c_, stream())
+            KernelTimer.run('conv_dgrad', gh.flops(), 'dmy_conv_dgrad', dt, ptr(dz), ptr(wts[h]), ptr(dx), h, N, H, W,
+                            C, C, c_, 1, 1, 1, 0, H, W, c_, stream(), tag=gh.tag(),
+                            nbytes=es * (M * c_ + c_ * C + (1 + h) * M * C))
+            _wgrad(dt, x, dz, c_, dws[h], gh, WGRAD_OIHW | WGRAD_ZEROED)
+        return (dx, dws[0], dws[1], *pg, None, None)
+
+
+def conv_pair_bn_act(x, conv1, bn1, act1, conv2, bn2, act2, out2=None):
+    sp1, sp2 = spec_for(conv1, 1, 0, act1, bn1), spec_for(conv2, 1, 0, act2, bn2)
+    return ConvPairFn.apply(x, conv1.weight, conv2.weight, bn1.weight, bn1.bias, bn2.weight, bn2.bias, (sp1, sp2),
+                            [out2] if out2 is not None else None)
+
+
+
 def _actbn_stats(z, g, spec, bn, train_bn):
     K, M, dev = g.K, g.M, z.device
     scale, shift = f32(K, dev), f32(K, dev)
diff --git a/dma-yolo_amd/dmayolo/models/common.py b/dma-yolo_amd/dmayolo/models/common.py
--- a/dma-yolo_amd/dmayolo/models/common.py
+++ b/dma-yolo_amd/dmayolo/models/common.py
@@ -203,9 +203,26 @@
                 a = blk(a)
             a = blocks[-1](a, out=cat[:, :c_])
             return self.cv3(Fn.ConcatFn.apply(None, 0.0, None, a, cat[:, c_:]), out=out)
+        inplace = seq or (getattr(self.m, 'dmy_out', False) and _INPLACE_CAT >= 2)
+        c1, c2 = self.cv1, self.cv2
+        if type(c1) is Conv and type(c2) is Conv and Fn.conv_pair_ok(
+                x, c1.conv, getattr(c1, 'bn', None), act_code(c1.act), c2.conv, getattr(c2, 'bn', None), act_code(c2.act)):
+            c_ = c1.conv.out_channels
+            cat = Fn.concat_buffer(x.shape[0], 2 * c_, x.shape[2], x.shape[3], x) if inplace else None
+            a, b = Fn.conv_pair_bn_act(x, c1.conv, c1.bn, act_code(c1.act), c2.conv, c2.bn, act_code(c2.act),
+                                       out2=cat[:, c_:] if inplace else None)
+            if not inplace:
+                a = self.m(a)
+            elif seq:
+                for blk in blocks[:-1]:
+                    a = blk(a)
+                a = blocks[-1](a, out=cat[:, :c_])
+            else:
+                a = self.m(a, out=cat[:, :c_])
+            return self.cv3(Fn.ConcatFn.apply(None, 0.0, None, a, b), out=out)
         sk = Fn.GradSink(2)
         a = self.cv1(x, xsink=sk)
-        if not seq and not (getattr(self.m, 'dmy_out', False) and _INPLACE_CAT >= 2):
+        if not inplace:
             return self.cv3(Fn.ConcatFn.apply(None, 0.0, None, self.m(a), self.cv2(x, xsink=sk)), out=out)
         c_ = a.shape[1]
         cat = Fn.concat_buffer(a.shape[0], 2 * c_, a.shape[2], a.shape[3], a)
diff --git a/include/dmayolo.h b/include/dmayolo.h
--- a/include/dmayolo.h
+++ b/include/dmayolo.h
@@ -32,6 +32,13 @@
                        const float* ca, const float* cb, const float* cc, void* dx, long bps, int accumulate,
                        float* dw, float* ws, long ws_elems, long M, int K, int C, void* stream);
 long dmy_conv1x1_bwd_bn_ws_elems(long M, int K, int C);
+int dmy_conv1x1_bwd_bn2_ok(long M, int K, int C, int ksplit, long dps, long dps1, long zps, long xps, long bps,
+                           const void* dy, const void* dy1, const void* z, const void* x, const void* dx);
+int dmy_conv1x1_bwd_bn2(const void* dy, long dps, const void* dy1, long dps1, int ksplit, const void* z, long zps,
+                        const void* x, long xps, const void* wt, const void* wt1, const float* scale,
+                        const float* shift, const float* mean, const float* invstd, int act, const float* ca,
+                        const float* cb, const float* cc, void* dx, long bps, int accumulate, float* dw, float* dw1,
+                        float* ws, long ws_elems, long M, int K, int C, void* stream);
 int dmy_conv_wgrad_ex(int dtype, const void* x, const void* dy, float* dw, int N, int H, int W, int C, long xps, int K,
                       int KH, int KW, int S, int P, int OH, int OW, long yps, int flags, void* stream);
 long dmy_conv_wgrad_ws_elems(int dtype, const void* x, const void* dy, int N, int H, int W, int C, long xps, int K,
@@ -153,6 +160,18 @@
 int dmy_bn_bwd_apply(int dtype, const void* z, long zps, const void* dy, long dps, const float* scale,
                      const float* shift, const float* mean, const float* invstd, int act, const float* ca,
                      const float* cb, const float* cc, void* dz, long dzps, long M, int C, void* stream);
+int dmy_bn_finalize_ld(const float* psum, const float* psq, int P, int C, int ld, double count, const float* gamma,
+                       const float* beta, float* running_mean, float* running_var, long long* num_batches_tracked,
+                       float momentum, float eps, int update, float* mean, float* invstd, float* scale, float* shift,
+                       void* stream);
+int dmy_bn_bwd_finalize_ld(const float* pdb, const float* pdg, int P, int C, int ld, double count, const float* gamma,
+                           const float* invstd, float* dgamma, float* dbeta, float* ca, float* cb, float* cc,
+                           void* stream);
+int dmy_bn_act_fwd2(int dtype, const void* z, long zps, const float* scale, const float* shift, int act, void* y0,
+                    long y0ps, void* y1, long y1ps, int csplit, long M, int C, void* stream);
+int dmy_bn_bwd_reduce2(int dtype, const void* z, long zps, const void* dy0, long dps0, const void* dy1, long dps1,
+                       int csplit, const float* scale, const float* shift, const float* mean, const float* invstd,
+                       int act, long M, int C, float* pdb, float* pdg, void* stream);
 int dmy_reduce_rows(const float* part, int P, int C, float* out, int accumulate, void* stream);
 int dmy_bn_reduce_rows(int dtype, const void* z, long zps, const void* dy, long dps, long M, int C);
 int dmy_colsum2_rows(long P);
```
